# tsadja/ShaSTA

Hardware: AMD Instinct MI355X
Metric: affinity frame-pairs/sec at N=M=500, F=256 (higher is better)
Workload: dtype f32; 1 GPU; synthetic N=M=500, F=256 (num_point 4 x C 64), nf=7: affinity forward from HBM-resident NHWC BEV maps (SURVEY 8a rows 4-16); max_obj=500, num_feats=7, num_point=4, arithmetic=f16x2, parallelism=replica x1

## Files before the change

### shasta_amd/csrc/pair.hip

```cpp
#include "stages.hpp"
#include "pair_lane.hpp"

namespace shasta {

struct PackArgs {
    shasta_linear fs[4], fd[3], rc[3], aff0;
    float* out;
    int N, nf, F;
};

__device__ __forceinline__ void layer_src(const PackArgs& a, int l, const float*& W, const float*& b, int& ldw) {
    const PairDims d(a.F);
    switch (l) {
        case L_FS2: W = a.fs[1].weight; b = a.fs[1].bias; ldw = d.H1; break;
        case L_FS3: W = a.fs[2].weight; b = a.fs[2].bias; ldw = d.H2; break;
        case L_FS4: W = a.fs[3].weight; b = a.fs[3].bias; ldw = d.H3; break;
        case L_RC2: W = a.rc[1].weight; b = a.rc[1].bias; ldw = d.R1; break;
        case L_RC3: W = a.rc[2].weight; b = a.rc[2].bias; ldw = d.R2; break;
        case L_FD2: W = a.fd[1].weight; b = a.fd[1].bias; ldw = 32; break;
        default:    W = a.fd[2].weight; b = a.fd[2].bias; ldw = 8; break;
    }
}

__global__ void pack_pair_weights_kernel(PackArgs a) {
    const PackedLayout P(a.N, a.nf, a.F);
    const PairDims d(a.F);
    const int tid = blockIdx.x * blockDim.x + threadIdx.x;
    const int nth = gridDim.x * blockDim.x;
    const int F = a.F, nf = a.nf;
    for (int l = 0; l < L_COUNT; ++l) {
        const LayerDesc L = layer_desc(F, l);
        const float *W, *b;
        int ldw;
        layer_src(a, l, W, b, ldw);
        const int nob = a4_nob(F, l), kg = a4_kg(F, l);
        float* o = a.out + P.a4 + a4_offset(F, l);
        for (int e = tid; e < nob * kg * 16; e += nth) {
            const int kk = e & 3, i = (e >> 2) & 3, g = (e >> 4) % kg, ob = (e >> 4) / kg;
            const int f = 4 * ob + i, k = 4 * g + kk;
            o[e] = (f < L.hout && k < L.kin) ? W[(size_t)f * ldw + k] : 0.0f;
        }
        for (int e = tid; e < nob * 4; e += nth) o[nob * kg * 16 + e] = e < L.hout ? b[e] : 0.0f;
    }
    const int E12 = P.E12;
    for (int e = tid; e < E12 * F; e += nth) {
        const int j = e / F, k = e % F;
        float wp, wc;
        if (j < d.H1) {
            wp = a.fs[0].weight[(size_t)j * 2 * F + k];
            wc = a.fs[0].weight[(size_t)j * 2 * F + F + k];
        } else {
            const size_t row = (size_t)(j - d.H1) * (2 * F + 2 * nf);
            wp = a.rc[0].weight[row + k];
            wc = a.rc[0].weight[row + F + nf + k];
        }
        a.out[P.wemb_prev + e] = wp;
        a.out[P.wemb_cur + e] = wc;
    }
    for (int e = tid; e < (E12 + 3) / 4 * 4; e += nth)
        a.out[P.bemb_cur + e] = e < d.H1 ? a.fs[0].bias[e] : (e < E12 ? a.rc[0].bias[e - d.H1] : 0.0f);
    for (int e = tid; e < (d.R1 + 32) * 8; e += nth) {
        const int j = e >> 3, c = e & 7;
        float wp = 0.0f, wc = 0.0f;
        if (c < nf) {
            if (j < d.R1) {
                const size_t row = (size_t)j * (2 * F + 2 * nf);
                wp = a.rc[0].weight[row + F + c];
                wc = a.rc[0].weight[row + 2 * F + nf + c];
            } else {
                const size_t row = (size_t)(j - d.R1) * (2 * nf);
                wp = a.fd[0].weight[row + c];
                wc = a.fd[0].weight[row + nf + c];
            }
        }
        a.out[P.wbox_prev + e] = wp;
        a.out[P.wbox_cur + e] = wc;
    }
    for (int e = tid; e < 32; e += nth) a.out[P.bbox_cur + e] = a.fd[0].bias[e];
    for (int e = tid; e < 128 * P.Dp; e += nth) {
        const int j = e / P.Dp, k = e % P.Dp;
        a.out[P.aff0 + e] = k < P.D ? a.aff0.weight[(size_t)j * P.D + k] : 0.0f;
    }
}

struct RowPrepArgs {
    const float* packed;
    const float* tab[2];
    float* emb[2];
    float* hand[2];
    float* denom;
    int B, T, N, nf, F, nrow_blocks, nhand_blocks, dblocks, dper;
};

template <int ND, int NF>
__device__ __forceinline__ void col_norm_block(const RowPrepArgs& a, int cb, int tid) {
    const int T = a.T, D = a.T, nf = NF ? NF : a.nf;
    const int b = cb / a.dblocks, dl = tid & 15, tg = tid >> 4;
    const int d0 = (cb % a.dblocks) * (16 * ND) + dl;
    float db[ND][7];
#pragma unroll
    for (int j = 0; j < ND; ++j) {
        const f32x4* h = reinterpret_cast<const f32x4*>(a.tab[1] + ((size_t)b * D + min(d0 + 16 * j, D - 1)) * 8);
        const f32x4 x = h[0], c = h[1];
        db[j][0] = x[0]; db[j][1] = x[1]; db[j][2] = x[2]; db[j][3] = x[3]; db[j][4] = c[0]; db[j][5] = c[1]; db[j][6] = c[2];
#pragma unroll
        for (int k = 0; k < 7; ++k)
            if (k >= nf) db[j][k] = 0.0f;
    }
    __shared__ __attribute__((aligned(16))) f32x4 sp[2 * 512];
    const f32x4* hp = reinterpret_cast<const f32x4*>(a.tab[0] + (size_t)b * T * 8);
    typedef float f2 __attribute__((ext_vector_type(2)));
    f2 ssq2[ND];
#pragma unroll
    for (int j = 0; j < ND; ++j) ssq2[j] = f2{0.0f, 0.0f};
    for (int t0 = 0; t0 < T; t0 += 512) {
        const int nt = min(512, T - t0);
        if (t0) __syncthreads();
        for (int e = tid; e < 2 * nt; e += 256) {
            f32x4 v = hp[(size_t)t0 * 2 + e];
            const int k0 = (e & 1) * 4;
#pragma unroll
            for (int q = 0; q < 4; ++q)
                if (k0 + q >= nf) v[q] = 0.0f;
            sp[e] = v;
        }
        __syncthreads();
        for (int t = tg; t < nt; t += 32) {
            const int tb = t + 16;
            const bool two = tb < nt;
            const f32x4 x0 = sp[2 * t], c0 = sp[2 * t + 1];
            const f32x4 x1 = sp[2 * (two ? tb : t)], c1 = sp[2 * (two ? tb : t) + 1];
            const f2 p[7] = {f2{x0[0], x1[0]}, f2{x0[1], x1[1]}, f2{x0[2], x1[2]}, f2{x0[3], x1[3]}, f2{c0[0], c1[0]}, f2{c0[1], c1[1]},
                             f2{c0[2], c1[2]}};
#pragma unroll
            for (int j = 0; j < ND; ++j) {
                f2 d2 = {0.0f, 0.0f};
#pragma unroll
                for (int k = 0; k < (NF ? NF : 7); ++k) {
                    const f2 df = p[k] - f2{db[j][k], db[j][k]};
                    d2 += df * df;
                }
                f2 sq = d2 * d2;
                if (!two) sq[1] = 0.0f;
                ssq2[j] += sq;
            }
        }
    }
    __shared__ float red4[ND][16][17];
#pragma unroll
    for (int j = 0; j < ND; ++j) red4[j][dl][tg] = ssq2[j][0] + ssq2[j][1];
    __syncthreads();
    if (tid < 16 * ND) {
        const int j = tid >> 4, l = tid & 15, dd = (cb % a.dblocks) * (16 * ND) + 16 * j + l;
        if (dd < D) {
            float tot = 0.0f;
#pragma unroll
            for (int i = 0; i < 16; ++i) tot += red4[j][l][i];
            a.denom[(size_t)b * D + dd] = fmaxf(sqrtf(tot), 1e-12f);
        }
    }
}

__global__ __launch_bounds__(256) void col_norm_kernel(RowPrepArgs a) { col_norm_block<4, 0>(a, blockIdx.x, threadIdx.x); }

__global__ __launch_bounds__(256) void row_prep_kernel(RowPrepArgs a) {
    const int tid = threadIdx.x;
    if ((int)blockIdx.x < a.nrow_blocks) {
        __shared__ __attribute__((aligned(16))) float wT[7 * 104];
        const PackedLayout P(a.N, a.nf, a.F);
        const PairDims d(a.F);
        const int J = d.R1 + 32;
        const int half = a.nrow_blocks / 2;
        const int which = (int)blockIdx.x >= half;
        const int side_row0 = (blockIdx.x - which * half) * 32;
        {
            const float* wb = a.packed + (which ? P.wbox_cur : P.wbox_prev);
            for (int e = tid; e < J * 8; e += 256) {
                const int j = e >> 3, c = e & 7;
                if (c < 7) wT[c * 104 + j] = wb[e];
            }
        }
        __syncthreads();
        const int q = tid & 31, nq = J / 4;
        for (int it = 0; it < 4; ++it) {
            const int row = side_row0 + it * 8 + (tid >> 5);
            if (row >= a.B * a.T) continue;
            float amax = 0.0f;
            if (q < nq) {
                const f32x4* bp = reinterpret_cast<const f32x4*>(a.tab[which] + (size_t)row * 8);
                const f32x4 b0 = bp[0], b1 = bp[1];
                const float bx[7] = {b0[0], b0[1], b0[2], b0[3], b1[0], b1[1], b1[2]};
                f32x4 s = {0.0f, 0.0f, 0.0f, 0.0f};
#pragma unroll
                for (int c = 0; c < 7; ++c) {
                    const f32x4 w4 = *reinterpret_cast<const f32x4*>(&wT[c * 104 + 4 * q]);
                    s[0] = fmaf(w4[0], bx[c], s[0]); s[1] = fmaf(w4[1], bx[c], s[1]);
                    s[2] = fmaf(w4[2], bx[c], s[2]); s[3] = fmaf(w4[3], bx[c], s[3]);
                }
                f32x4* e = reinterpret_cast<f32x4*>(a.emb[which] + (size_t)row * d.ET + d.H1 + 4 * q);
                const int j = 4 * q;
                if (j < d.R1) {
                    f32x4 v = *e;
                    s[0] += v[0]; s[1] += v[1]; s[2] += v[2]; s[3] += v[3];
                } else if (which) {
                    const f32x4 bb = *reinterpret_cast<const f32x4*>(a.packed + P.bbox_cur + (j - d.R1));
                    s[0] += bb[0]; s[1] += bb[1]; s[2] += bb[2]; s[3] += bb[3];
                }
                *e = s;
                amax = absmax_keep_nan(absmax_keep_nan(fabsf(s[0]), fabsf(s[1])), absmax_keep_nan(fabsf(s[2]), fabsf(s[3])));
            } else {
                const f32x4* e = reinterpret_cast<const f32x4*>(a.emb[which] + (size_t)row * d.ET);
                for (int c4 = q - nq; c4 < d.H1 / 4; c4 += 32 - nq) {
                    const f32x4 v = e[c4];
                    amax = absmax_keep_nan(amax, absmax_keep_nan(absmax_keep_nan(fabsf(v[0]), fabsf(v[1])), absmax_keep_nan(fabsf(v[2]), fabsf(v[3]))));
                }
            }
#pragma unroll
            for (int off = 16; off > 0; off >>= 1) amax = absmax_keep_nan(amax, __shfl_xor(amax, off, 64));
            if (q == 0) a.hand[which][(size_t)row * 16 + 13] = amax;
        }
        return;
    }
    if ((int)blockIdx.x < a.nrow_blocks + a.nhand_blocks) {
        const int item = (blockIdx.x - a.nrow_blocks) * 256 + tid;
        if (item >= 2 * a.B * a.T) return;
        const int which = item / (a.B * a.T), row = item % (a.B * a.T);
        const f32x4* bp = reinterpret_cast<const f32x4*>(a.tab[which] + (size_t)row * 8);
        const f32x4 b0 = bp[0], b1 = bp[1];
        f32x4* h = reinterpret_cast<f32x4*>(a.hand[which] + (size_t)row * 16);
        const int nf = a.nf;
        h[0] = f32x4{b0[0], nf > 1 ? b0[1] : 0.0f, nf > 2 ? b0[2] : 0.0f, nf > 3 ? b0[3] : 0.0f};
        h[1] = f32x4{nf > 4 ? b1[0] : 0.0f, nf > 5 ? b1[1] : 0.0f, nf > 6 ? b1[2] : 0.0f, 0.0f};
        h[2] = f32x4{logf(b0[3] + 1e-10f), logf(b1[0] + 1e-10f), logf(b1[1] + 1e-10f), cosf(b1[2])};
        a.hand[which][(size_t)row * 16 + 12] = sinf(b1[2]);
        return;
    }
    const int cb = blockIdx.x - a.nrow_blocks - a.nhand_blocks;
    if (a.dper == 4) {
        col_norm_block<4, 0>(a, cb, tid);
    } else {
        col_norm_block<1, 0>(a, cb, tid);
    }
}

template <int F, int WPB, int DT>
struct PairMfma4Lds {
    static constexpr int US = PairDims(F).ET + 4;
    static constexpr int RING = 3 * (64 / DT);
    static constexpr int uc = 0;
    static constexpr int a4 = uc + DT * US;
    static constexpr int up = a4 + pad4(a4_total(F));
    static constexpr size_t bytes = (size_t)(up + WPB * RING * UP_SLOT) * sizeof(float);
};
static_assert(PairMfma4Lds<64, 8, 64>::bytes == 49760 && PairMfma4Lds<64, 8, 32>::bytes == 63584 &&
              PairMfma4Lds<256, 8, 64>::bytes == 66800 && PairMfma4Lds<256, 8, 32>::bytes == 74480 &&
              PairMfma4Lds<320, 8, 64>::bytes == 74336 && PairMfma4Lds<320, 8, 32>::bytes == 79968, "the sizes the launcher spelt out before");

template <int F, int WPB, int DT = 64>
__global__ __launch_bounds__(64 * WPB) __attribute__((amdgpu_waves_per_eu(4))) void pair_mfma4_kernel(const float* __restrict__ packed, const float* __restrict__ UP,
                                                         const float* __restrict__ UC, const float* __restrict__ hand_prev,
                                                         const float* __restrict__ hand_det, const float* __restrict__ denom,
                                                         float* __restrict__ residual, int T, int D, int ld, int nf,
                                                         int TW) {
    constexpr PairDims dm(F);
    constexpr int H1 = dm.H1, R1 = dm.R1, ET = dm.ET;
    using Lds = PairMfma4Lds<F, WPB, DT>;
    constexpr int US = Lds::US, RING = Lds::RING;
    static_assert(DT == 64 || DT == 32, "64 detections x 1 track or 32 detections x 2 tracks per wave");
    constexpr int TPI = 64 / DT;
    extern __shared__ __attribute__((aligned(16))) float s_dyn4[];
    float* s_uc = s_dyn4 + Lds::uc;
    float* s_a4 = s_dyn4 + Lds::a4;
    float* s_up = s_dyn4 + Lds::up;
    const int tid = threadIdx.x, lane = tid & 63;
    const int wid = __builtin_amdgcn_readfirstlane(tid >> 6);
    const int dlane = lane & (DT - 1), th = lane / DT;
    int lbx, lby, b;
    xcd_logical_block(lbx, lby, b);
    const int d0 = lbx * DT;
    const int d = d0 + dlane, dcl = min(d, D - 1);
    {
        const f32x4* src = reinterpret_cast<const f32x4*>(UC);
#pragma unroll 4
        for (int e = tid; e < DT * (ET / 4); e += 64 * WPB) {
            const int r = e / (ET / 4), c = e - r * (ET / 4);
            *reinterpret_cast<f32x4*>(&s_uc[r * US + 4 * c]) = src[((size_t)b * D + min(d0 + r, D - 1)) * (ET / 4) + c];
        }
        a4_stage<F, 64 * WPB>(packed, s_a4, tid);
    }
    float hd[12];
    (void)load_hand_det(hand_det + ((size_t)b * D + dcl) * 16, hd);
    const float dnm = denom[(size_t)b * D + dcl], rdn = 1.0f / dnm;
    __syncthreads();
    const float* ucrow = s_uc + dlane * US;
    const A4Lane a4l(s_a4, lane);

    const int t_beg = (lby * WPB + wid) * TW;
    const int t_end = min(T, t_beg + TW);
    float* my_up = s_up + wid * (RING * UP_SLOT);
    const bool hp_lane = lane >= ET / 4 && lane < ET / 4 + 4;
    const int up_lane = 4 * min(lane, ET / 4 - 1), hp_off = 4 * (lane - ET / 4);
    auto dma_up = [&](int row, int slot) {
        const size_t r = (size_t)b * T + min(row, T - 1);
        const float* src = hp_lane ? hand_prev + r * 16 + hp_off : UP + r * ET + up_lane;
        __builtin_amdgcn_global_load_lds((const __attribute__((address_space(1))) void*)src,
                                         (__attribute__((address_space(3))) void*)(my_up + slot * UP_SLOT), 16, 0, 0);
    };
    if (t_beg < t_end) {
#pragma unroll
        for (int i = 0; i < 2 * TPI; ++i) dma_up(t_beg + i, i);
    }
    for (int t = t_beg; t < t_end; t += TPI) {
        asm volatile("s_waitcnt vmcnt(0)" ::: "memory");
#pragma unroll
        for (int i = 0; i < TPI; ++i) dma_up(t + 2 * TPI + i, (t - t_beg + 2 * TPI + i) % RING);
        const int tt = t + th;
        unsigned upo = (unsigned)(unsigned long long)(my_up + ((t - t_beg + th) % RING) * UP_SLOT);
        asm volatile("" : "+v"(upo));
        const lfloat* up = (const lfloat*)(unsigned long long)upo;
        float hp[16];
        {
            const f32x4 h0 = *reinterpret_cast<const lf32x4*>(up + ET), h1 = *reinterpret_cast<const lf32x4*>(up + ET + 4),
                        h2 = *reinterpret_cast<const lf32x4*>(up + ET + 8), h3 = *reinterpret_cast<const lf32x4*>(up + ET + 12);
#pragma unroll
            for (int k = 0; k < 4; ++k) {
                hp[k] = h0[k];
                hp[4 + k] = h1[k];
                hp[8 + k] = h2[k];
                hp[12 + k] = h3[k];
            }
        }
        const lfloat *arow, *abias;
        a4l.per_track(arow, abias);

        auto layer12 = [&](auto tag, int seg, f32x4* acc) {
            using AL = decltype(tag);
            a4_init<AL>(abias, acc);
#pragma unroll
            for (int kg = 0; kg < AL::KG; ++kg) {
                const f32x4 u = *reinterpret_cast<const f32x4*>(ucrow + seg + 4 * kg);
                const f32x4 upv = *reinterpret_cast<const lf32x4*>(up + seg + 4 * kg);
                f32x4 a4[AL::NOB];
#pragma unroll
                for (int ob = 0; ob < AL::NOB; ++ob) a4[ob] = *reinterpret_cast<const lf32x4*>(arow + AL::OFF + (ob * AL::KG + kg) * 16);
#pragma unroll
                for (int kk = 0; kk < 4; ++kk) {
                    if (4 * kg + kk < AL::KIN) {
                        const float h = relu_nan(upv[kk] + u[kk]);
#pragma unroll
                        for (int ob = 0; ob < AL::NOB; ++ob) acc[ob] = MFMA4(a4[ob][kk], h, acc[ob]);
                    }
                }
            }
        };
        f32x4 a_rc2[A4<F, L_RC2>::NOB], a_rc3[A4<F, L_RC3>::NOB];
        f32x4 a_fs2[A4<F, L_FS2>::NOB], a_fs3[A4<F, L_FS3>::NOB], a_fs4[A4<F, L_FS4>::NOB];
        f32x4 a_fd2[A4<F, L_FD2>::NOB], a_fd3[A4<F, L_FD3>::NOB];
        layer12(A4<F, L_RC2>{}, H1, a_rc2);
        layer12(A4<F, L_FS2>{}, 0, a_fs2);
        layer12(A4<F, L_FD2>{}, H1 + R1, a_fd2);
        a4_layer<A4<F, L_RC3>, A4_RELU_NAN>(arow, abias, a_rc2, a_rc3);
        a4_layer<A4<F, L_FS3>, A4_RELU_NAN>(arow, abias, a_fs2, a_fs3);
        a4_layer<A4<F, L_FD3>, A4_RELU_NAN>(arow, abias, a_fd2, a_fd3);
        a4_layer<A4<F, L_FS4>, A4_RELU_NAN>(arow, abias, a_fs3, a_fs4);

        const float dist = hand_dist(hp, hd, dnm, rdn);
        const float res = pair_combine(a_rc3[0], a_fd3[0][0], dist, a_fs4[0][0]);
        if (d < D && tt < t_end) residual[((size_t)b * T + tt) * ld + d] = res;
    }
}

int pair_residual(const shasta_weights* w, const float* packed, int B, const float* feat, const float* prev_feat,
                  const float* det_tab, const float* prev_tab, float* residual, int ld, void* ws, size_t ws_bytes,
                  hipStream_t st, hipEvent_t ev0, hipEvent_t ev1) {
    const int N = w->max_obj, F = w->feat_dim, nf = w->num_feats, T = N + 2, D = N + 2;
    const PairDims d(F);
    const PackedLayout P(N, nf, F);
    const PairWs L(B, N, F);
    if (ws_bytes < L.total) {
        set_error_msg("pair_residual: workspace too small");
        return SHASTA_E_WORKSPACE;
    }
    if (B == 0) return SHASTA_OK;
    char* base = static_cast<char*>(ws);
    float* UP = reinterpret_cast<float*>(base + L.up);
    float* UC = reinterpret_cast<float*>(base + L.uc);
    float* hand_prev = reinterpret_cast<float*>(base + L.hand_prev);
    float* hand_det = reinterpret_cast<float*>(base + L.hand_det);
    float* denom = reinterpret_cast<float*>(base + L.denom);

    const bool gemm_f32 = (w->options & SHASTA_OPT_F32_EMBED_GEMM) != 0;
    const bool fused = B * T >= 8192 && !gemm_f32 && embed_rows_serves(F) && ((uintptr_t)feat | (uintptr_t)prev_feat) % 16 == 0;
    int rc;
    if (fused)
        rc = launch_embed_rows(w, packed, prev_feat, feat, prev_tab, det_tab, UP, UC, hand_prev, hand_det, B * T, st);
    else
        rc = launch_gemm_nt_dual(prev_feat, packed + P.wemb_prev, nullptr, UP, feat, packed + P.wemb_cur, packed + P.bemb_cur, UC, F, F,
                                 d.ET, B * T, P.E12, F, 0, st);
    if (rc) return rc;
    RowPrepArgs rp;
    rp.packed = packed;
    rp.tab[0] = prev_tab;
    rp.tab[1] = det_tab;
    rp.emb[0] = UP;
    rp.emb[1] = UC;
    rp.hand[0] = hand_prev;
    rp.hand[1] = hand_det;
    rp.denom = denom;
    rp.B = B;
    rp.T = T;
    rp.N = N;
    rp.nf = nf;
    rp.F = F;
    rp.nrow_blocks = fused ? 0 : 2 * cdiv(B * T, 32);
    rp.nhand_blocks = cdiv(2 * B * T, 256);
    rp.dper = cdiv(D, 16) * B >= 2048 ? 4 : 1;
    rp.dblocks = cdiv(D, 16 * rp.dper);
    if (rp.dper == 4) {
        hipLaunchKernelGGL(row_prep_kernel, dim3(rp.nrow_blocks + rp.nhand_blocks), dim3(256), 0, st, rp);
        rc = check_launch("row_prep");
        if (rc) return rc;
        hipLaunchKernelGGL(col_norm_kernel, dim3(rp.dblocks * B), dim3(256), 0, st, rp);
        rc = check_launch("col_norm");
    } else {
        hipLaunchKernelGGL(row_prep_kernel, dim3(rp.nrow_blocks + rp.nhand_blocks + rp.dblocks * B), dim3(256), 0, st, rp);
        rc = check_launch("row_prep");
    }
    if (rc) return rc;
    if ((w->options & SHASTA_OPT_F16X2_PAIR) && F == 256) {
        if (ev0) (void)hipEventRecord(ev0, st);
        const bool grid = (w->options & SHASTA_OPT_F16GRID_PAIR) != 0 && fused;
        rc = launch_pair_f16(packed, packed + P.p16, UP, UC, hand_prev, hand_det, denom, residual, B, T, D, ld, nf, grid, st);
        if (ev1) (void)hipEventRecord(ev1, st);
        return rc;
    }
    if ((w->options & SHASTA_OPT_F16X2_PAIR) && pair_f16w_serves(F)) {
        if (ev0) (void)hipEventRecord(ev0, st);
        rc = launch_pair_f16w(packed, packed + P.p16w, UP, UC, hand_prev, hand_det, denom, residual, B, T, D, ld, F, st);
        if (ev1) (void)hipEventRecord(ev1, st);
        if (rc != SHASTA_E_UNSUPPORTED) return rc;
    }
    constexpr int wpb = 8;
    const double fill64 = (double)D / (64.0 * cdiv(D, 64)), fill32 = (double)D / (32.0 * cdiv(D, 32));
    const int dt = fill32 > 1.1 * fill64 ? 32 : 64, tpi = 64 / dt;
    int ny = 1;
    while ((long)B * cdiv(D, dt) * ny < 1024 && cdiv(T, wpb * ny * 2) >= 2 * tpi) ny *= 2;
    while ((long)B * cdiv(D, dt) * ny < 256 && cdiv(T, wpb * ny * 2) >= tpi) ny *= 2;
    const int tw = cdiv(cdiv(T, wpb * ny), tpi) * tpi;
    dim3 grid(cdiv(D, dt), cdiv(T, wpb * tw), B);
#define SHASTA_LAUNCH_PAIR4_DT(FF, DD)                                                                                                    \
    do {                                                                                                                                  \
        constexpr size_t lds = PairMfma4Lds<FF, wpb, DD>::bytes;                                                                          \
        if (lds > 64 * 1024)                                                                                                              \
            (void)hipFuncSetAttribute((const void*)pair_mfma4_kernel<FF, wpb, DD>, hipFuncAttributeMaxDynamicSharedMemorySize, (int)lds); \
        hipLaunchKernelGGL((pair_mfma4_kernel<FF, wpb, DD>), grid, dim3(64 * wpb), lds, st, packed, UP, UC, hand_prev, hand_det, denom,   \
                           residual, T, D, ld, nf, tw);                                                                                   \
    } while (0)
#define SHASTA_LAUNCH_PAIR4(FF)                 \
    do {                                        \
        if (dt == 32) SHASTA_LAUNCH_PAIR4_DT(FF, 32); \
        else SHASTA_LAUNCH_PAIR4_DT(FF, 64);    \
    } while (0)
    if (ev0) (void)hipEventRecord(ev0, st);
    switch (F) {
        case 64: SHASTA_LAUNCH_PAIR4(64); break;
        case 256: SHASTA_LAUNCH_PAIR4(256); break;
        case 320: SHASTA_LAUNCH_PAIR4(320); break;
        default: set_error_msg("pair_residual: feat_dim must be 64, 256 or 320"); return SHASTA_E_ARG;
    }
    if (ev1) (void)hipEventRecord(ev1, st);
#undef SHASTA_LAUNCH_PAIR4_DT
#undef SHASTA_LAUNCH_PAIR4
    return check_launch("pair_mfma4");
}

int pack_weights(const shasta_weights* w, float* packed, hipStream_t st) {
    PackArgs a;
    for (int i = 0; i < 4; ++i) a.fs[i] = w->fuse_shape[i];
    for (int i = 0; i < 3; ++i) a.fd[i] = w->fuse_det[i];
    for (int i = 0; i < 3; ++i) a.rc[i] = w->res_coeff[i];
    a.aff0 = w->aff[0];
    a.out = packed;
    a.N = w->max_obj;
    a.nf = w->num_feats;
    a.F = w->feat_dim;
    hipLaunchKernelGGL(pack_pair_weights_kernel, dim3(256), dim3(256), 0, st, a);
    int rc = check_launch("pack_pair_weights");
    if (rc) return rc;
    const PackedLayout P(w->max_obj, w->num_feats, w->feat_dim);
    if ((rc = aff_pieces_pack(w, packed + P.affp, st))) return rc;
    if ((rc = aff_f16_pack(w, packed + P.aff16, st))) return rc;
    if (w->feat_dim == 256 && (rc = pair_f16_pack(w, packed + P.p16, st))) return rc;
    if (pair_f16w_serves(w->feat_dim) && (rc = pair_f16w_pack(w, packed + P.p16w, st))) return rc;
    if (embed_rows_serves(w->feat_dim) && (rc = embed_pack(w, packed, st))) return rc;
    return rc;
}

}
```

### shasta_amd/csrc/pair_f16.hip

```cpp
#include "stages.hpp"
#include "pair_lane.hpp"
#include "pieces.hpp"

namespace shasta {


constexpr int P16_FRAG_DW = 2 * 4 * 64 * 4;

__global__ __launch_bounds__(256) void pair_f16_pack_kernel(PairF16PackArgs a) {
    __shared__ float red[3][4];
    __shared__ int ex[3];
    const int tid = threadIdx.x;
    const float* W[3] = {a.w_fs2, a.w_rc2, a.w_fd2};
    const int cnt[3] = {16 * 32, 16 * 64, 8 * 32};
    pair2_range_exponents(W, cnt, a.out, P16_FRAG_DW, red, ex);
    const int lane = tid & 63, frag = tid >> 6;
    const int i = lane & 15, kb = lane >> 4;
    const int mlp = frag == 0 ? 0 : frag == 3 ? 2 : 1;
    const int rows = mlp == 2 ? 8 : 16, kin = mlp == 1 ? 64 : 32, ks = frag == 2 ? 1 : 0;
    float v[8];
#pragma unroll
    for (int j = 0; j < 8; ++j) v[j] = i < rows ? __builtin_ldexpf(W[mlp][i * kin + 32 * ks + 8 * kb + j], ex[mlp]) : 0.0f;
    store_weight_pieces(v, a.out, 4, frag, lane);
}

int pair_f16_pack(const shasta_weights* w, float* out, hipStream_t st) {
    hipLaunchKernelGGL(pair_f16_pack_kernel, dim3(1), dim3(256), 0, st, pair_f16_pack_args(w, out));
    return check_launch("pair_f16_pack");
}

constexpr int PF_TS = 44;
constexpr int GR_ROW = 136;

template <int WPB, bool GRID>
struct PairF16Lds {
    static constexpr int US = PairDims(256).ET + 4;
    static constexpr int uc = 0;
    static constexpr int ucl = uc + 64 * (GR_ROW / 2);
    static constexpr int a4 = uc + (GRID ? 2 * 64 * (GR_ROW / 2) : 64 * US);
    static constexpr int up = a4 + pad4(a4_total(256));
    static constexpr int tr = up + WPB * 3 * UP_SLOT;
    static constexpr int upp = tr + WPB * 64 * PF_TS;
    static constexpr size_t bytes = (size_t)(upp + (GRID ? WPB * 128 : 0)) * sizeof(float);
};
static_assert(PairF16Lds<8, false>::bytes == 156912 && PairF16Lds<8, true>::bytes == 162032, "the sizes the launcher spelt out before");


template <int WPB, bool GRID>
__global__ __launch_bounds__(64 * WPB) void pair_f16_kernel(const float* __restrict__ packed, const uint32_t* __restrict__ p16,
                                                       const float* __restrict__ UP, const float* __restrict__ UC,
                                                       const float* __restrict__ hand_prev, const float* __restrict__ hand_det,
                                                       const float* __restrict__ denom, float* __restrict__ residual, int T,
                                                       int D, int ld, int nf, int TWG, int TA, int TB) {
    constexpr int F = 256;
    constexpr PairDims dm(F);
    constexpr int ET = dm.ET;
    static_assert(dm.H1 == 32 && dm.R1 == 64 && ET == 128 && dm.H2 == 16 && dm.R2 == 16, "pair_f16_kernel is laid out for F = 256");
    using Lds = PairF16Lds<WPB, GRID>;
    constexpr int US = Lds::US;
    extern __shared__ __attribute__((aligned(16))) float s_dynh[];
    float* s_uc = s_dynh + Lds::uc;
    float* s_a4 = s_dynh + Lds::a4;
    float* s_up = s_dynh + Lds::up;
    float* s_tr = s_dynh + Lds::tr;
    uint32_t* s_uch = reinterpret_cast<uint32_t*>(s_dynh + Lds::uc);
    uint32_t* s_ucl = reinterpret_cast<uint32_t*>(s_dynh + Lds::ucl);
    uint32_t* s_upp = reinterpret_cast<uint32_t*>(s_dynh + Lds::upp);
    const int tid = threadIdx.x, lane = tid & 63;
    const int wid = __builtin_amdgcn_readfirstlane(tid >> 6);
    int lbx, by, b;
    xcd_logical_block(lbx, by, b);
    const int d0 = lbx * 64;
    const int d = d0 + lane, dcl = min(d, D - 1);
    {
        if constexpr (!GRID) {
            const f32x4* src = reinterpret_cast<const f32x4*>(UC);
#pragma unroll 4
            for (int e = tid; e < 64 * (ET / 4); e += 64 * WPB) {
                const int r = e / (ET / 4), c = e - r * (ET / 4);
                const int cp = (((c >> 1) & 1) << 4) | (((c >> 2) & 1) << 3) | ((c >> 3) << 1) | (c & 1);
                *reinterpret_cast<f32x4*>(&s_uc[r * US + 4 * cp]) = src[((size_t)b * D + min(d0 + r, D - 1)) * (ET / 4) + c];
            }
        }
        a4_stage<F, 64 * WPB>(packed, s_a4, tid);
    }
    float hd[12];
    float mc = load_hand_det(hand_det + ((size_t)b * D + dcl) * 16, hd);
#pragma unroll
    for (int off = 32; off > 0; off >>= 1) mc = absmax_keep_nan(mc, __shfl_xor(mc, off, 64));
    const float dnm = denom[(size_t)b * D + dcl], rdn = 1.0f / dnm;
    int ge[3] = {0, 0, 0};
    bool grid_finite = true;
    if constexpr (GRID) {
        float mcr[3], mur[3] = {0.0f, 0.0f, 0.0f};
        {
            const float* h = hand_det + ((size_t)b * D + dcl) * 16;
            mcr[0] = h[14];
            mcr[1] = h[15];
            mcr[2] = h[13];
        }
        const int tw0 = by * TWG, tw1 = min(T, tw0 + TWG);
        for (int t = tw0 + tid; t < tw1; t += 64 * WPB) {
            const float* h = hand_prev + ((size_t)b * T + t) * 16;
            mur[0] = absmax_keep_nan(mur[0], h[14]);
            mur[1] = absmax_keep_nan(mur[1], h[15]);
            mur[2] = absmax_keep_nan(mur[2], h[13]);
        }
#pragma unroll
        for (int r = 0; r < 3; ++r)
#pragma unroll
            for (int off = 32; off > 0; off >>= 1) {
                mcr[r] = absmax_keep_nan(mcr[r], __shfl_xor(mcr[r], off, 64));
                mur[r] = absmax_keep_nan(mur[r], __shfl_xor(mur[r], off, 64));
            }
        float* red = s_tr;
        if (lane == 0) {
            red[wid * 3 + 0] = mur[0];
            red[wid * 3 + 1] = mur[1];
            red[wid * 3 + 2] = mur[2];
        }
        __syncthreads();
#pragma unroll
        for (int r = 0; r < 3; ++r) {
            float m = red[r];
            for (int w = 1; w < WPB; ++w) m = absmax_keep_nan(m, red[w * 3 + r]);
            const float bound = (m + mcr[r]) * 1.002f;
            grid_finite = grid_finite && (bound < INFINITY);
            ge[r] = range_exponent_bits(__float_as_uint(bound)) - 3;
        }
        __syncthreads();
        const f32x4* src = reinterpret_cast<const f32x4*>(UC);
        for (int e = tid; e < 64 * (ET / 4); e += 64 * WPB) {
            const int r = e / (ET / 4), c = e - r * (ET / 4);
            const f32x4 v = src[((size_t)b * D + min(d0 + r, D - 1)) * (ET / 4) + c];
            const int ex = c < 8 ? ge[0] : c < 24 ? ge[1] : ge[2];
            _Float16 hh[4], ll[4];
#pragma unroll
            for (int q = 0; q < 4; ++q) {
                const float sv = __builtin_ldexpf(v[q], ex), hi = rintf(sv);
                hh[q] = (_Float16)hi;
                ll[q] = (_Float16)(rintf((sv - hi) * 2048.0f) * (1.0f / 2048.0f));
            }
            typedef uint32_t pu2 __attribute__((ext_vector_type(2)));
            typedef _Float16 ph2t __attribute__((ext_vector_type(2)));
            *reinterpret_cast<pu2*>(s_uch + r * (GR_ROW / 2) + 2 * c) =
                pu2{__builtin_bit_cast(uint32_t, ph2t{hh[0], hh[1]}), __builtin_bit_cast(uint32_t, ph2t{hh[2], hh[3]})};
            *reinterpret_cast<pu2*>(s_ucl + r * (GR_ROW / 2) + 2 * c) =
                pu2{__builtin_bit_cast(uint32_t, ph2t{ll[0], ll[1]}), __builtin_bit_cast(uint32_t, ph2t{ll[2], ll[3]})};
        }
    }
    u32x4 wh[4], wl[4];
#pragma unroll
    for (int f = 0; f < 4; ++f) {
        wh[f] = reinterpret_cast<const u32x4*>(p16)[(0 * 4 + f) * 64 + lane];
        wl[f] = reinterpret_cast<const u32x4*>(p16)[(1 * 4 + f) * 64 + lane];
    }
    const int ew_fs = reinterpret_cast<const int*>(p16)[P16_FRAG_DW + 0], ew_rc = reinterpret_cast<const int*>(p16)[P16_FRAG_DW + 1],
              ew_fd = reinterpret_cast<const int*>(p16)[P16_FRAG_DW + 2];
    __syncthreads();
    const A4Lane a4l(s_a4, lane);
    const f32x4 zero4 = {0, 0, 0, 0};
    const int p = lane & 15, kb = lane >> 4;
    float* my_tr = s_tr + wid * (64 * PF_TS);

    const int t_beg = by * TWG + (wid < 4 ? wid * TA : 4 * TA + (wid - 4) * TB);
    const int t_end = min(min(T, (by + 1) * TWG), t_beg + (wid < 4 ? TA : TB));
    float* my_up = s_up + wid * (3 * UP_SLOT);
    const bool hp_lane = lane >= ET / 4 && lane < ET / 4 + 4;
    const int up_lane = 4 * min(lane, ET / 4 - 1), hp_off = 4 * (lane - ET / 4);
    auto dma_up = [&](int row, int slot) {
        const size_t r = (size_t)b * T + min(row, T - 1);
        const float* src = hp_lane ? hand_prev + r * 16 + hp_off : UP + r * ET + up_lane;
        __builtin_amdgcn_global_load_lds((const __attribute__((address_space(1))) void*)src,
                                         (__attribute__((address_space(3))) void*)(my_up + slot * UP_SLOT), 16, 0, 0);
    };
    if (t_beg < t_end) {
        dma_up(t_beg, 0);
        dma_up(t_beg + 1, 1);
    }
    for (int t = t_beg; t < t_end; ++t) {
        asm volatile("s_waitcnt vmcnt(0)" ::: "memory");
        dma_up(t + 2, (t - t_beg + 2) % 3);
        unsigned upo = (unsigned)(unsigned long long)(my_up + ((t - t_beg) % 3) * UP_SLOT);
        asm volatile("" : "+v"(upo));
        const lfloat* up = (const lfloat*)(unsigned long long)upo;
        float hp[16];
        {
            const f32x4 h0 = *reinterpret_cast<const lf32x4*>(up + ET), h1 = *reinterpret_cast<const lf32x4*>(up + ET + 4),
                        h2 = *reinterpret_cast<const lf32x4*>(up + ET + 8), h3 = *reinterpret_cast<const lf32x4*>(up + ET + 12);
#pragma unroll
            for (int k = 0; k < 4; ++k) {
                hp[k] = h0[k];
                hp[4 + k] = h1[k];
                hp[8 + k] = h2[k];
                hp[12 + k] = h3[k];
            }
        }
        typedef _Float16 ph2 __attribute__((ext_vector_type(2)));
        bool finite_bound;
        int e1 = 0;
        f32x2 cs2 = {0.0f, 0.0f};
        const f32x2 c14 = {16384.0f, 16384.0f};
        f32x2 upv[GRID ? 1 : 16];
        u32x4 uph[GRID ? 4 : 1], upl[GRID ? 4 : 1];
        if constexpr (!GRID) {
            const float bound = hp[13] + mc;
            finite_bound = bound < INFINITY;
            e1 = range_exponent_bits(__float_as_uint(bound));
            const float cs = __builtin_ldexpf(1.0f, e1 - 14);
            cs2 = f32x2{cs, cs};
#pragma unroll
            for (int s = 0; s < 4; ++s) {
                const f32x4 a = *reinterpret_cast<const lf32x4*>(up + 32 * s + 8 * kb), c = *reinterpret_cast<const lf32x4*>(up + 32 * s + 8 * kb + 4);
                upv[4 * s] = f32x2{a[0], a[1]} * cs2;
                upv[4 * s + 1] = f32x2{a[2], a[3]} * cs2;
                upv[4 * s + 2] = f32x2{c[0], c[1]} * cs2;
                upv[4 * s + 3] = f32x2{c[2], c[3]} * cs2;
            }
        } else {
            finite_bound = grid_finite;
            uint32_t* my_p = s_upp + wid * 128;
            {
                typedef __attribute__((address_space(3))) f32x2 lf32x2;
                const f32x2 v = *reinterpret_cast<const lf32x2*>(up + 2 * lane);
                const int ex = lane < 16 ? ge[0] : lane < 48 ? ge[1] : ge[2];
                const float s0 = __builtin_ldexpf(v[0], ex), s1 = __builtin_ldexpf(v[1], ex);
                const float h0 = rintf(s0), h1v = rintf(s1);
                const ph2 hh = {(_Float16)h0, (_Float16)h1v};
                const ph2 ll = {(_Float16)(rintf((s0 - h0) * 2048.0f) * (1.0f / 2048.0f)), (_Float16)(rintf((s1 - h1v) * 2048.0f) * (1.0f / 2048.0f))};
                my_p[lane] = __builtin_bit_cast(uint32_t, hh);
                my_p[64 + lane] = __builtin_bit_cast(uint32_t, ll);
            }
#pragma unroll
            for (int s = 0; s < 4; ++s) {
                uph[s] = *reinterpret_cast<const u32x4*>(my_p + 16 * s + 4 * kb);
                upl[s] = *reinterpret_cast<const u32x4*>(my_p + 64 + 16 * s + 4 * kb);
            }
        }
        auto load_uc = [&](int sub, f32x4 (&u)[8]) {
            if constexpr (GRID) {
                const uint32_t* hr = s_uch + (16 * sub + p) * (GR_ROW / 2) + 4 * kb;
                const uint32_t* lr = s_ucl + (16 * sub + p) * (GR_ROW / 2) + 4 * kb;
#pragma unroll
                for (int s = 0; s < 4; ++s) {
                    u[s] = __builtin_bit_cast(f32x4, *reinterpret_cast<const u32x4*>(hr + 16 * s));
                    u[4 + s] = __builtin_bit_cast(f32x4, *reinterpret_cast<const u32x4*>(lr + 16 * s));
                }
                return;
            }
            const float* ucr = s_uc + (16 * sub + p) * US + ((kb & 1) << 6) + ((kb >> 1) << 5);
#pragma unroll
            for (int s = 0; s < 4; ++s) {
                u[2 * s] = *reinterpret_cast<const f32x4*>(ucr + 8 * s);
                u[2 * s + 1] = *reinterpret_cast<const f32x4*>(ucr + 8 * s + 4);
            }
        };
        auto cut = [&](const f32x4 (&u)[8], u32x4 (&xh)[4], u32x4 (&xl)[4]) {
            if constexpr (GRID) {
                const _Float16 m1 = (_Float16)-1.0f;
                const f16x8 neg1 = {m1, m1, m1, m1, m1, m1, m1, m1};
#pragma unroll
                for (int s = 0; s < 4; ++s) {
                    const f16x8 h = __builtin_bit_cast(f16x8, u[s]) + __builtin_bit_cast(f16x8, uph[s]);
                    const f16x8 l = __builtin_bit_cast(f16x8, u[4 + s]) + __builtin_bit_cast(f16x8, upl[s]);
                    const f16x8 h2 = __builtin_elementwise_max(h, neg1);
                    const f16x8 l2 = __builtin_elementwise_max(l, -h2);
                    xh[s] = __builtin_bit_cast(u32x4, h2);
                    xl[s] = __builtin_bit_cast(u32x4, l2);
                }
                return;
            }
#pragma unroll
            for (int s = 0; s < 4; ++s) {
#pragma unroll
                for (int j2 = 0; j2 < 2; ++j2) {
                    const f32x4 uu = u[2 * s + j2];
                    const f32x2 sa = fma2_relu01(f32x2{uu[0], uu[1]}, cs2, upv[4 * s + 2 * j2]) * c14;
                    const f32x2 sb = fma2_relu01(f32x2{uu[2], uu[3]}, cs2, upv[4 * s + 2 * j2 + 1]) * c14;
                    const uint32_t hA = cvt_f16x2(sa[0], sa[1]), hB = cvt_f16x2(sb[0], sb[1]);
                    xh[s][2 * j2] = hA;
                    xh[s][2 * j2 + 1] = hB;
                    xl[s][2 * j2] = cvt_f16x2(f16_res_lo(sa[0], hA), f16_res_hi(sa[1], hA));
                    xl[s][2 * j2 + 1] = cvt_f16x2(f16_res_lo(sb[0], hB), f16_res_hi(sb[1], hB));
                }
            }
        };
        auto mma = [&](const u32x4 (&xh)[4], const u32x4 (&xl)[4], f32x4& a_fs, f32x4& a_rc, f32x4& a_fd) {
            a_fs = a_rc = a_fd = zero4;
            a_fs = mfma_16x16x32_f16(wl[0], xh[0], a_fs);
            a_rc = mfma_16x16x32_f16(wl[1], xh[1], a_rc);
            a_fd = mfma_16x16x32_f16(wl[3], xh[3], a_fd);
            a_fs = mfma_16x16x32_f16(wh[0], xl[0], a_fs);
            a_rc = mfma_16x16x32_f16(wh[1], xl[1], a_rc);
            a_fd = mfma_16x16x32_f16(wh[3], xl[3], a_fd);
            a_rc = mfma_16x16x32_f16(wl[2], xh[2], a_rc);
            a_fs = mfma_16x16x32_f16(wh[0], xh[0], a_fs);
            a_fd = mfma_16x16x32_f16(wh[3], xh[3], a_fd);
            a_rc = mfma_16x16x32_f16(wh[2], xl[2], a_rc);
            a_rc = mfma_16x16x32_f16(wh[1], xh[1], a_rc);
            a_rc = mfma_16x16x32_f16(wh[2], xh[2], a_rc);
        };
        auto store = [&](int sub, const f32x4& a_fs, const f32x4& a_rc, const f32x4& a_fd) {
            float* row = my_tr + (16 * sub + p) * PF_TS + 4 * kb;
            *reinterpret_cast<f32x4*>(row) = a_rc;
            *reinterpret_cast<f32x4*>(row + 16) = a_fs;
            if (kb < 2) *reinterpret_cast<f32x4*>(row + 32) = a_fd;
        };
        {
            f32x4 ua[8], ub[8];
            u32x4 xha[4], xla[4], xhb[4], xlb[4];
            f32x4 fsA, rcA, fdA, fsB, rcB, fdB;
            load_uc(0, ua);
            load_uc(1, ub);
            cut(ua, xha, xla);
            load_uc(2, ua);
            cut(ub, xhb, xlb);
            mma(xha, xla, fsA, rcA, fdA);
            store(0, fsA, rcA, fdA);
            load_uc(3, ub);
            cut(ua, xha, xla);
            mma(xhb, xlb, fsB, rcB, fdB);
            store(1, fsB, rcB, fdB);
            cut(ub, xhb, xlb);
            mma(xha, xla, fsA, rcA, fdA);
            store(2, fsA, rcA, fdA);
            mma(xhb, xlb, fsB, rcB, fdB);
            store(3, fsB, rcB, fdB);
        }
        const lfloat *arow, *abias;
        a4l.per_track(arow, abias);
        const float i_rc = __builtin_ldexpf(1.0f, -((GRID ? ge[1] : e1) + ew_rc)), i_fs = __builtin_ldexpf(1.0f, -((GRID ? ge[0] : e1) + ew_fs)),
                    i_fd = __builtin_ldexpf(1.0f, -((GRID ? ge[2] : e1) + ew_fd));
        f32x4 a_rc2[4], a_fs2[4], a_fd2[2];
        {
            const float* mine = my_tr + lane * PF_TS;
            const float* b_rc = s_a4 + A4<F, L_RC2>::OFF + A4<F, L_RC2>::BIAS;
            const float* b_fs = s_a4 + A4<F, L_FS2>::OFF + A4<F, L_FS2>::BIAS;
            const float* b_fd = s_a4 + A4<F, L_FD2>::OFF + A4<F, L_FD2>::BIAS;
#pragma unroll
            for (int g = 0; g < 4; ++g) {
                a_rc2[g] = a4_descale_relu(*reinterpret_cast<const f32x4*>(mine + 4 * g), i_rc, *reinterpret_cast<const f32x4*>(b_rc + 4 * g));
                a_fs2[g] = a4_descale_relu(*reinterpret_cast<const f32x4*>(mine + 16 + 4 * g), i_fs, *reinterpret_cast<const f32x4*>(b_fs + 4 * g));
            }
#pragma unroll
            for (int g = 0; g < 2; ++g)
                a_fd2[g] = a4_descale_relu(*reinterpret_cast<const f32x4*>(mine + 32 + 4 * g), i_fd, *reinterpret_cast<const f32x4*>(b_fd + 4 * g));
        }
        asm volatile("" : "+v"(a_rc2[0]), "+v"(a_rc2[1]), "+v"(a_rc2[2]), "+v"(a_rc2[3]), "+v"(a_fs2[0]), "+v"(a_fs2[1]), "+v"(a_fs2[2]),
                     "+v"(a_fs2[3]), "+v"(a_fd2[0]), "+v"(a_fd2[1]));
        f32x4 a_rc3[A4<F, L_RC3>::NOB], a_fs3[A4<F, L_FS3>::NOB], a_fs4[A4<F, L_FS4>::NOB], a_fd3[A4<F, L_FD3>::NOB];
        {
            using RC = A4<F, L_RC3>;
            using FS = A4<F, L_FS3>;
            using FD = A4<F, L_FD3>;
            static_assert(RC::NOB == 1 && FS::NOB == 2 && FD::NOB == 1 && RC::KG == 4 && FS::KG == 4 && FD::KG == 2, "F = 256");
            a4_init<RC>(abias, a_rc3);
            a4_init<FS>(abias, a_fs3);
            a4_init<FD>(abias, a_fd3);
#pragma unroll
            for (int kg = 0; kg < 4; ++kg) {
                const f32x4 w_rc = *reinterpret_cast<const lf32x4*>(arow + RC::OFF + kg * 16);
                const f32x4 w_f0 = *reinterpret_cast<const lf32x4*>(arow + FS::OFF + kg * 16);
                const f32x4 w_f1 = *reinterpret_cast<const lf32x4*>(arow + FS::OFF + (FS::KG + kg) * 16);
                f32x4 w_fd = zero4;
                if (kg < 2) w_fd = *reinterpret_cast<const lf32x4*>(arow + FD::OFF + kg * 16);
#pragma unroll
                for (int kk = 0; kk < 4; ++kk) {
                    a_rc3[0] = MFMA4(w_rc[kk], a_rc2[kg][kk], a_rc3[0]);
                    a_fs3[0] = MFMA4(w_f0[kk], a_fs2[kg][kk], a_fs3[0]);
                    a_fs3[1] = MFMA4(w_f1[kk], a_fs2[kg][kk], a_fs3[1]);
                    if (kg < 2) a_fd3[0] = MFMA4(w_fd[kk], a_fd2[kg][kk], a_fd3[0]);
                }
            }
        }
        a4_layer<A4<F, L_FS4>, A4_RELU_FMAX>(arow, abias, a_fs3, a_fs4);

        const float dist = hand_dist(hp, hd, dnm, rdn);
        const float res = pair_combine(a_rc3[0], a_fd3[0][0], dist, a_fs4[0][0]);
        if (d < D) residual[((size_t)b * T + t) * ld + d] = finite_bound ? res : __builtin_nanf("");
    }
}

int launch_pair_f16(const float* packed, const float* p16, const float* UP, const float* UC, const float* hand_prev,
                    const float* hand_det, const float* denom, float* residual, int B, int T, int D, int ld, int nf, bool grid,
                    hipStream_t st) {
    constexpr int wpb = 8;
    int ny = 1;
    while ((long)B * cdiv(D, 64) * ny < 512 && cdiv(T, wpb * ny * 2) >= 2) ny *= 2;
    const int twg = cdiv(cdiv(T, ny), wpb) * wpb;
    int ta = twg / wpb, tb = ta;
    if (wpb == 8) {
        const int per_simd = twg / 4;
        ta = (per_simd * 1000 + (1000 + 615) / 2) / (1000 + 615);
        tb = per_simd - ta;
    }
    const size_t lds = grid ? PairF16Lds<wpb, true>::bytes : PairF16Lds<wpb, false>::bytes;
    dim3 grd(cdiv(D, 64), cdiv(T, twg), B);
    if (grid) {
        (void)hipFuncSetAttribute((const void*)pair_f16_kernel<wpb, true>, hipFuncAttributeMaxDynamicSharedMemorySize, (int)lds);
        hipLaunchKernelGGL((pair_f16_kernel<wpb, true>), grd, dim3(64 * wpb), lds, st, packed, reinterpret_cast<const uint32_t*>(p16), UP, UC,
                           hand_prev, hand_det, denom, residual, T, D, ld, nf, twg, ta, tb);
    } else {
        (void)hipFuncSetAttribute((const void*)pair_f16_kernel<wpb, false>, hipFuncAttributeMaxDynamicSharedMemorySize, (int)lds);
        hipLaunchKernelGGL((pair_f16_kernel<wpb, false>), grd, dim3(64 * wpb), lds, st, packed, reinterpret_cast<const uint32_t*>(p16), UP, UC,
                           hand_prev, hand_det, denom, residual, T, D, ld, nf, twg, ta, tb);
    }
    return check_launch("pair_f16");
}

}
```

### shasta_amd/csrc/stages.hpp

```cpp
#pragma once
#include "common.hpp"
#include "pair_layout.hpp"

namespace shasta {

size_t bev_absmax_slot_bytes(int items);
int launch_absmax_finalize(const unsigned* slots, unsigned* out, int items, hipStream_t st);
int launch_bev_gather(const float* bev, int B, int H, int W, int C, const float* boxes, int N, int box_stride, int box_batch_stride,
                      int num_point, float pc_x0, float pc_y0, float vs_x, float vs_y, float out_stride, float* out, int out_row_stride,
                      int out_batch_stride, unsigned* absmax, hipStream_t st, const float* bev2 = nullptr, const float* boxes2 = nullptr,
                      float* out2 = nullptr, unsigned* absmax2 = nullptr);

int launch_gemm_nt_dual(const float* A0, const float* W0, const float* bias0, float* C0, const float* A1, const float* W1,
                        const float* bias1, float* C1, int lda, int ldw, int ldc, int M, int N, int K, int act, hipStream_t st);
int launch_gemm_nt_quad(const float* const A[4], const float* const W[4], const float* const bias[4], float* const C[4], int lda,
                        int ldw, int ldc, int M, int N, int K, int act, hipStream_t st);
bool gemm_nt_quad_direct_ok(const float* const A[4], const float* const W[4], int lda, int ldw, int K);

int launch_anchor_l1_mfma(const float* const W[4], const float* feat, const float* prev_feat, float* part, int H, int K, int B,
                          int x_batch_stride, int* ks_out, hipStream_t st);

int launch_x_maxima(const float* feat, const float* prev_feat, int K, int B, int x_batch_stride, unsigned* xmax, hipStream_t st);
int launch_w_maxima(const float* const W[4], int H, int K, unsigned* wmax, float* sumabs, hipStream_t st);
size_t precut_image_bytes(int H, int K);
int launch_precut_weights(const float* const W[4], const unsigned* wmax, void* img, int H, int K, hipStream_t st);
size_t anchor_split_workspace_bytes(int B, int K);
bool anchor_split_serves(int B, int K, int x_batch_stride);
void launch_split_x(const float* feat, const float* prev_feat, void* xs, int K, int B, int x_batch_stride, int np, const unsigned* xmax,
                    bool precut, hipStream_t st);
void launch_anchor_l1_split(const float* const W[4], const void* xs, float* part, int H, int K, int B, int* ks_out, int np,
                            const unsigned* wmax, const void* wimg, hipStream_t st);

int anchor_shape(const shasta_weights* w, int B, float* feat, float* prev_feat, void* ws, size_t ws_bytes, hipStream_t st,
                 hipEvent_t ev0, hipEvent_t ev1, const unsigned* wmax, bool xmax_ready);
bool anchor_shape_uses_xmax(const shasta_weights* w, int B);
int anchor_boxes(const shasta_weights* w, int B, float* det_boxes, const float* prev_det_boxes, int box_stride, float* det_tab,
                 float* prev_tab, float* hid_ws, hipStream_t st, float* anchors_out);
bool anchor_stage_fused_serves(const shasta_weights* w, int B);
int anchor_stage_fused(const shasta_weights* w, int B, float* feat, float* prev_feat, float* det_boxes, const float* prev_det_boxes,
                       int box_stride, float* det_tab, float* prev_tab, void* ws, size_t ws_bytes, hipStream_t st, hipEvent_t ev0,
                       hipEvent_t ev1, const unsigned* wmax, bool xmax_ready, float* anchors_out);

int pair_f16_pack(const shasta_weights* w, float* out, hipStream_t st);
int launch_pair_f16(const float* packed, const float* p16, const float* UP, const float* UC, const float* hand_prev,
                    const float* hand_det, const float* denom, float* residual, int B, int T, int D, int ld, int nf, bool grid,
                    hipStream_t st);
bool pair_f16w_serves(int F);
int pair_f16w_pack(const shasta_weights* w, float* out, hipStream_t st);
int launch_pair_f16w(const float* packed, const float* p16, const float* UP, const float* UC, const float* hand_prev,
                     const float* hand_det, const float* denom, float* residual, int B, int T, int D, int ld, int F, hipStream_t st);

int embed_pack(const shasta_weights* w, float* packed, hipStream_t st);
bool embed_rows_serves(int F);
int launch_embed_rows(const shasta_weights* w, const float* packed, const float* prev_feat, const float* feat, const float* prev_tab,
                      const float* det_tab, float* UP, float* UC, float* hand_prev, float* hand_det, int M, hipStream_t st);

int pair_residual(const shasta_weights* w, const float* packed, int B, const float* feat, const float* prev_feat, const float* det_tab,
                  const float* prev_tab, float* residual, int ld, void* ws, size_t ws_bytes, hipStream_t st, hipEvent_t ev0,
                  hipEvent_t ev1);
int pack_weights(const shasta_weights* w, float* packed, hipStream_t st);

int aff_pieces_pack(const shasta_weights* w, float* out, hipStream_t st);
int aff_f16_pack(const shasta_weights* w, float* out, hipStream_t st);
bool aff_pieces_serves(int D);
int launch_aff_pieces(const shasta_weights* w, const float* packed_pieces, const float* residual, int ld, float* matched, int ldm,
                      float* m1, int M, hipStream_t st);
int launch_aff_frame(const shasta_weights* w, const float* packed_pieces, const float* residual, int ld, float* matched, int ldm, float* m1,
                     float* m2, int B, void* ws, hipStream_t st);
int launch_aff_frame16(const shasta_weights* w, const float* packed16, const float* residual, int ld, float* matched, int ldm, float* m1,
                       float* m2, int B, void* ws, hipStream_t st);

int aff_status(const shasta_weights* w, int B, int ld, const void* ws, int* status, hipStream_t st);
int aff_softmax(const shasta_weights* w, const float* packed, int B, const float* residual, int ld, float* m1, float* m2,
                float* matched_out, void* ws, size_t ws_bytes, hipStream_t st);


inline size_t ws_take(size_t& o, size_t bytes) {
    const size_t at = o;
    o += align_up(bytes, 256);
    return at;
}

struct AnchorShapeWs {
    size_t part, hidden, xs, xmax, wmax, slots, total;
    AnchorShapeWs(int B, int N, int F) {
        const size_t H = (size_t)N * F / 64;
        size_t o = 0;
        part = ws_take(o, (size_t)64 * B * 4 * H * sizeof(float));
        hidden = ws_take(o, (size_t)B * 4 * H * sizeof(float));
        xs = ws_take(o, anchor_split_workspace_bytes(B, N * F));
        xmax = ws_take(o, (size_t)2 * B * sizeof(unsigned));
        wmax = ws_take(o, (size_t)4 * H * sizeof(unsigned));
        slots = o;
        total = o + bev_absmax_slot_bytes(2 * B);
    }
};

struct AnchorBoxesWs {
    size_t hid, x7, total;
    AnchorBoxesWs(int B, int N) {
        const int HD = 7 * N / 32;
        size_t o = 0;
        hid = ws_take(o, (size_t)B * 4 * (HD > 1 ? HD : 1) * sizeof(float));
        x7 = ws_take(o, (size_t)2 * B * pad4(7 * N) * sizeof(float));
        total = o;
    }
};

struct PairWs {
    size_t up, uc, hand_prev, hand_det, denom, total;
    PairWs(int B, int N, int F) {
        const size_t rows = (size_t)B * (N + 2);
        size_t o = 0;
        up = ws_take(o, rows * PairDims(F).ET * sizeof(float));
        uc = ws_take(o, rows * PairDims(F).ET * sizeof(float));
        hand_prev = ws_take(o, rows * 16 * sizeof(float));
        hand_det = ws_take(o, rows * 16 * sizeof(float));
        denom = ws_take(o, rows * sizeof(float));
        total = o;
    }
};

struct AffWs {
    size_t matched, ctrl, part, total;
    AffWs(int B, int N) {
        const int T = N + 2;
        size_t o = 0;
        matched = ws_take(o, (size_t)B * T * pad4(T) * sizeof(float));
        ctrl = ws_take(o, (size_t)(B + 2) * sizeof(unsigned));
        part = ws_take(o, (size_t)B * cdiv(T, 64) * 1024 * sizeof(float));
        total = o;
    }
};

}
```

Measured before the change: 64280 frame-pairs/s.

## Make f16 pair kernel persistent with per-XCD atomic tile tickets

Turns the f16x2 pair kernel into a persistent kernel with one workgroup per CU when there are more tiles than CUs. Workgroups take tiles from eight atomic ticket counters, one per XCD-sized slice, and steal from other slices once their own runs out. Packed weights are staged into LDS once per workgroup instead of once per tile. The cost is a global atomic and an extra barrier per tile, plus counters that row_prep must reset on every call.

```diff
diff --git a/shasta_amd/csrc/pair.hip b/shasta_amd/csrc/pair.hip
--- a/shasta_amd/csrc/pair.hip
+++ b/shasta_amd/csrc/pair.hip
@@ -89,6 +89,7 @@
     float* emb[2];
     float* hand[2];
     float* denom;
+    unsigned* tickets;
     int B, T, N, nf, F, nrow_blocks, nhand_blocks, dblocks, dper;
 };
 
@@ -223,6 +224,7 @@
     }
     if ((int)blockIdx.x < a.nrow_blocks + a.nhand_blocks) {
         const int item = (blockIdx.x - a.nrow_blocks) * 256 + tid;
+        if (item < 8) a.tickets[item] = 0;
         if (item >= 2 * a.B * a.T) return;
         const int which = item / (a.B * a.T), row = item % (a.B * a.T);
         const f32x4* bp = reinterpret_cast<const f32x4*>(a.tab[which] + (size_t)row * 8);
@@ -407,6 +409,7 @@
     rp.hand[0] = hand_prev;
     rp.hand[1] = hand_det;
     rp.denom = denom;
+    rp.tickets = reinterpret_cast<unsigned*>(base + L.tickets);
     rp.B = B;
     rp.T = T;
     rp.N = N;
@@ -430,7 +433,7 @@
     if ((w->options & SHASTA_OPT_F16X2_PAIR) && F == 256) {
         if (ev0) (void)hipEventRecord(ev0, st);
         const bool grid = (w->options & SHASTA_OPT_F16GRID_PAIR) != 0 && fused;
-        rc = launch_pair_f16(packed, packed + P.p16, UP, UC, hand_prev, hand_det, denom, residual, B, T, D, ld, nf, grid, st);
+        rc = launch_pair_f16(packed, packed + P.p16, UP, UC, hand_prev, hand_det, denom, residual, B, T, D, ld, nf, grid, rp.tickets, st);
         if (ev1) (void)hipEventRecord(ev1, st);
         return rc;
     }
diff --git a/shasta_amd/csrc/pair_f16.hip b/shasta_amd/csrc/pair_f16.hip
--- a/shasta_amd/csrc/pair_f16.hip
+++ b/shasta_amd/csrc/pair_f16.hip
@@ -41,9 +41,10 @@
     static constexpr int up = a4 + pad4(a4_total(256));
     static constexpr int tr = up + WPB * 3 * UP_SLOT;
     static constexpr int upp = tr + WPB * 64 * PF_TS;
-    static constexpr size_t bytes = (size_t)(upp + (GRID ? WPB * 128 : 0)) * sizeof(float);
+    static constexpr int ctl = upp + (GRID ? WPB * 128 : 0);
+    static constexpr size_t bytes = (size_t)(ctl + 4) * sizeof(float);
 };
-static_assert(PairF16Lds<8, false>::bytes == 156912 && PairF16Lds<8, true>::bytes == 162032, "the sizes the launcher spelt out before");
+static_assert(PairF16Lds<8, false>::bytes == 156928 && PairF16Lds<8, true>::bytes == 162048, "one workgroup per CU (160 KB)");
 
 
 template <int WPB, bool GRID>
@@ -51,7 +52,8 @@
                                                        const float* __restrict__ UP, const float* __restrict__ UC,
                                                        const float* __restrict__ hand_prev, const float* __restrict__ hand_det,
                                                        const float* __restrict__ denom, float* __restrict__ residual, int T,
-                                                       int D, int ld, int nf, int TWG, int TA, int TB) {
+                                                       int D, int ld, int nf, int TWG, int TA, int TB, unsigned* __restrict__ tickets,
+                                                       int NX, int NY, int NT) {
     constexpr int F = 256;
     constexpr PairDims dm(F);
     constexpr int ET = dm.ET;
@@ -66,89 +68,14 @@
     uint32_t* s_uch = reinterpret_cast<uint32_t*>(s_dynh + Lds::uc);
     uint32_t* s_ucl = reinterpret_cast<uint32_t*>(s_dynh + Lds::ucl);
     uint32_t* s_upp = reinterpret_cast<uint32_t*>(s_dynh + Lds::upp);
+    unsigned* s_ctl = reinterpret_cast<unsigned*>(s_dynh + Lds::ctl);
     const int tid = threadIdx.x, lane = tid & 63;
     const int wid = __builtin_amdgcn_readfirstlane(tid >> 6);
-    int lbx, by, b;
-    xcd_logical_block(lbx, by, b);
-    const int d0 = lbx * 64;
-    const int d = d0 + lane, dcl = min(d, D - 1);
-    {
-        if constexpr (!GRID) {
-            const f32x4* src = reinterpret_cast<const f32x4*>(UC);
-#pragma unroll 4
-            for (int e = tid; e < 64 * (ET / 4); e += 64 * WPB) {
-                const int r = e / (ET / 4), c = e - r * (ET / 4);
-                const int cp = (((c >> 1) & 1) << 4) | (((c >> 2) & 1) << 3) | ((c >> 3) << 1) | (c & 1);
-                *reinterpret_cast<f32x4*>(&s_uc[r * US + 4 * cp]) = src[((size_t)b * D + min(d0 + r, D - 1)) * (ET / 4) + c];
-            }
-        }
-        a4_stage<F, 64 * WPB>(packed, s_a4, tid);
-    }
-    float hd[12];
-    float mc = load_hand_det(hand_det + ((size_t)b * D + dcl) * 16, hd);
-#pragma unroll
-    for (int off = 32; off > 0; off >>= 1) mc = absmax_keep_nan(mc, __shfl_xor(mc, off, 64));
-    const float dnm = denom[(size_t)b * D + dcl], rdn = 1.0f / dnm;
-    int ge[3] = {0, 0, 0};
-    bool grid_finite = true;
-    if constexpr (GRID) {
-        float mcr[3], mur[3] = {0.0f, 0.0f, 0.0f};
-        {
-            const float* h = hand_det + ((size_t)b * D + dcl) * 16;
-            mcr[0] = h[14];
-            mcr[1] = h[15];
-            mcr[2] = h[13];
-        }
-        const int tw0 = by * TWG, tw1 = min(T, tw0 + TWG);
-        for (int t = tw0 + tid; t < tw1; t += 64 * WPB) {
-            const float* h = hand_prev + ((size_t)b * T + t) * 16;
-            mur[0] = absmax_keep_nan(mur[0], h[14]);
-            mur[1] = absmax_keep_nan(mur[1], h[15]);
-            mur[2] = absmax_keep_nan(mur[2], h[13]);
-        }
-#pragma unroll
-        for (int r = 0; r < 3; ++r)
-#pragma unroll
-            for (int off = 32; off > 0; off >>= 1) {
-                mcr[r] = absmax_keep_nan(mcr[r], __shfl_xor(mcr[r], off, 64));
-                mur[r] = absmax_keep_nan(mur[r], __shfl_xor(mur[r], off, 64));
-            }
-        float* red = s_tr;
-        if (lane == 0) {
-            red[wid * 3 + 0] = mur[0];
-            red[wid * 3 + 1] = mur[1];
-            red[wid * 3 + 2] = mur[2];
-        }
-        __syncthreads();
-#pragma unroll
-        for (int r = 0; r < 3; ++r) {
-            float m = red[r];
-            for (int w = 1; w < WPB; ++w) m = absmax_keep_nan(m, red[w * 3 + r]);
-            const float bound = (m + mcr[r]) * 1.002f;
-            grid_finite = grid_finite && (bound < INFINITY);
-            ge[r] = range_exponent_bits(__float_as_uint(bound)) - 3;
-        }
-        __syncthreads();
-        const f32x4* src = reinterpret_cast<const f32x4*>(UC);
-        for (int e = tid; e < 64 * (ET / 4); e += 64 * WPB) {
-            const int r = e / (ET / 4), c = e - r * (ET / 4);
-            const f32x4 v = src[((size_t)b * D + min(d0 + r, D - 1)) * (ET / 4) + c];
-            const int ex = c < 8 ? ge[0] : c < 24 ? ge[1] : ge[2];
-            _Float16 hh[4], ll[4];
-#pragma unroll
-            for (int q = 0; q < 4; ++q) {
-                const float sv = __builtin_ldexpf(v[q], ex), hi = rintf(sv);
-                hh[q] = (_Float16)hi;
-                ll[q] = (_Float16)(rintf((sv - hi) * 2048.0f) * (1.0f / 2048.0f));
-            }
-            typedef uint32_t pu2 __attribute__((ext_vector_type(2)));
-            typedef _Float16 ph2t __attribute__((ext_vector_type(2)));
-            *reinterpret_cast<pu2*>(s_uch + r * (GR_ROW / 2) + 2 * c) =
-                pu2{__builtin_bit_cast(uint32_t, ph2t{hh[0], hh[1]}), __builtin_bit_cast(uint32_t, ph2t{hh[2], hh[3]})};
-            *reinterpret_cast<pu2*>(s_ucl + r * (GR_ROW / 2) + 2 * c) =
-                pu2{__builtin_bit_cast(uint32_t, ph2t{ll[0], ll[1]}), __builtin_bit_cast(uint32_t, ph2t{ll[2], ll[3]})};
-        }
-    }
+    const bool persistent = tickets != nullptr;
+    const unsigned per = (unsigned)NT >> 3;
+    unsigned tq = blockIdx.x & 7, tk = 0;
+    if (persistent && tid == 0) tk = __hip_atomic_fetch_add(tickets + tq, 1u, __ATOMIC_RELAXED, __HIP_MEMORY_SCOPE_AGENT);
+    a4_stage<F, 64 * WPB>(packed, s_a4, tid);
     u32x4 wh[4], wl[4];
 #pragma unroll
     for (int f = 0; f < 4; ++f) {
@@ -157,233 +84,334 @@
     }
     const int ew_fs = reinterpret_cast<const int*>(p16)[P16_FRAG_DW + 0], ew_rc = reinterpret_cast<const int*>(p16)[P16_FRAG_DW + 1],
               ew_fd = reinterpret_cast<const int*>(p16)[P16_FRAG_DW + 2];
-    __syncthreads();
     const A4Lane a4l(s_a4, lane);
     const f32x4 zero4 = {0, 0, 0, 0};
     const int p = lane & 15, kb = lane >> 4;
     float* my_tr = s_tr + wid * (64 * PF_TS);
-
-    const int t_beg = by * TWG + (wid < 4 ? wid * TA : 4 * TA + (wid - 4) * TB);
-    const int t_end = min(min(T, (by + 1) * TWG), t_beg + (wid < 4 ? TA : TB));
     float* my_up = s_up + wid * (3 * UP_SLOT);
     const bool hp_lane = lane >= ET / 4 && lane < ET / 4 + 4;
     const int up_lane = 4 * min(lane, ET / 4 - 1), hp_off = 4 * (lane - ET / 4);
-    auto dma_up = [&](int row, int slot) {
-        const size_t r = (size_t)b * T + min(row, T - 1);
-        const float* src = hp_lane ? hand_prev + r * 16 + hp_off : UP + r * ET + up_lane;
-        __builtin_amdgcn_global_load_lds((const __attribute__((address_space(1))) void*)src,
-                                         (__attribute__((address_space(3))) void*)(my_up + slot * UP_SLOT), 16, 0, 0);
-    };
-    if (t_beg < t_end) {
-        dma_up(t_beg, 0);
-        dma_up(t_beg + 1, 1);
-    }
-    for (int t = t_beg; t < t_end; ++t) {
-        asm volatile("s_waitcnt vmcnt(0)" ::: "memory");
-        dma_up(t + 2, (t - t_beg + 2) % 3);
-        unsigned upo = (unsigned)(unsigned long long)(my_up + ((t - t_beg) % 3) * UP_SLOT);
-        asm volatile("" : "+v"(upo));
-        const lfloat* up = (const lfloat*)(unsigned long long)upo;
-        float hp[16];
+    for (;;) {
+        int lbx, by, b;
+        if (persistent) {
+            if (tid == 0) {
+                for (int tries = 0; tk >= (tq == 7 ? (unsigned)NT - 7 * per : per) && tries < 7; ++tries) {
+                    tq = (tq + 1) & 7;
+                    tk = __hip_atomic_fetch_add(tickets + tq, 1u, __ATOMIC_RELAXED, __HIP_MEMORY_SCOPE_AGENT);
+                }
+                s_ctl[0] = tk < (tq == 7 ? (unsigned)NT - 7 * per : per) ? tq * per + tk : (unsigned)NT;
+            }
+            asm volatile("s_waitcnt vmcnt(0)" ::: "memory");
+            __syncthreads();
+            const int L = __builtin_amdgcn_readfirstlane(s_ctl[0]);
+            if (L >= NT) break;
+            lbx = L % NX;
+            by = (L / NX) % NY;
+            b = L / (NX * NY);
+        } else {
+            xcd_logical_block(lbx, by, b);
+        }
+        const int d0 = lbx * 64;
+        const int d = d0 + lane, dcl = min(d, D - 1);
         {
-            const f32x4 h0 = *reinterpret_cast<const lf32x4*>(up + ET), h1 = *reinterpret_cast<const lf32x4*>(up + ET + 4),
-                        h2 = *reinterpret_cast<const lf32x4*>(up + ET + 8), h3 = *reinterpret_cast<const lf32x4*>(up + ET + 12);
-#pragma unroll
-            for (int k = 0; k < 4; ++k) {
-                hp[k] = h0[k];
-                hp[4 + k] = h1[k];
-                hp[8 + k] = h2[k];
-                hp[12 + k] = h3[k];
-            }
-        }
-        typedef _Float16 ph2 __attribute__((ext_vector_type(2)));
-        bool finite_bound;
-        int e1 = 0;
-        f32x2 cs2 = {0.0f, 0.0f};
-        const f32x2 c14 = {16384.0f, 16384.0f};
-        f32x2 upv[GRID ? 1 : 16];
-        u32x4 uph[GRID ? 4 : 1], upl[GRID ? 4 : 1];
-        if constexpr (!GRID) {
-            const float bound = hp[13] + mc;
-            finite_bound = bound < INFINITY;
-            e1 = range_exponent_bits(__float_as_uint(bound));
-            const float cs = __builtin_ldexpf(1.0f, e1 - 14);
-            cs2 = f32x2{cs, cs};
-#pragma unroll
-            for (int s = 0; s < 4; ++s) {
-                const f32x4 a = *reinterpret_cast<const lf32x4*>(up + 32 * s + 8 * kb), c = *reinterpret_cast<const lf32x4*>(up + 32 * s + 8 * kb + 4);
-                upv[4 * s] = f32x2{a[0], a[1]} * cs2;
-                upv[4 * s + 1] = f32x2{a[2], a[3]} * cs2;
-                upv[4 * s + 2] = f32x2{c[0], c[1]} * cs2;
-                upv[4 * s + 3] = f32x2{c[2], c[3]} * cs2;
-            }
-        } else {
-            finite_bound = grid_finite;
-            uint32_t* my_p = s_upp + wid * 128;
+            if constexpr (!GRID) {
+                const f32x4* src = reinterpret_cast<const f32x4*>(UC);
+#pragma unroll 4
+                for (int e = tid; e < 64 * (ET / 4); e += 64 * WPB) {
+                    const int r = e / (ET / 4), c = e - r * (ET / 4);
+                    const int cp = (((c >> 1) & 1) << 4) | (((c >> 2) & 1) << 3) | ((c >> 3) << 1) | (c & 1);
+                    *reinterpret_cast<f32x4*>(&s_uc[r * US + 4 * cp]) = src[((size_t)b * D + min(d0 + r, D - 1)) * (ET / 4) + c];
+                }
+            }
+        }
+        float hd[12];
+        float mc = load_hand_det(hand_det + ((size_t)b * D + dcl) * 16, hd);
+#pragma unroll
+        for (int off = 32; off > 0; off >>= 1) mc = absmax_keep_nan(mc, __shfl_xor(mc, off, 64));
+        const float dnm = denom[(size_t)b * D + dcl], rdn = 1.0f / dnm;
+        int ge[3] = {0, 0, 0};
+        bool grid_finite = true;
+        if constexpr (GRID) {
+            float mcr[3], mur[3] = {0.0f, 0.0f, 0.0f};
             {
-                typedef __attribute__((address_space(3))) f32x2 lf32x2;
-                const f32x2 v = *reinterpret_cast<const lf32x2*>(up + 2 * lane);
-                const int ex = lane < 16 ? ge[0] : lane < 48 ? ge[1] : ge[2];
-                const float s0 = __builtin_ldexpf(v[0], ex), s1 = __builtin_ldexpf(v[1], ex);
-                const float h0 = rintf(s0), h1v = rintf(s1);
-                const ph2 hh = {(_Float16)h0, (_Float16)h1v};
-                const ph2 ll = {(_Float16)(rintf((s0 - h0) * 2048.0f) * (1.0f / 2048.0f)), (_Float16)(rintf((s1 - h1v) * 2048.0f) * (1.0f / 2048.0f))};
-                my_p[lane] = __builtin_bit_cast(uint32_t, hh);
-                my_p[64 + lane] = __builtin_bit_cast(uint32_t, ll);
-            }
-#pragma unroll
-            for (int s = 0; s < 4; ++s) {
-                uph[s] = *reinterpret_cast<const u32x4*>(my_p + 16 * s + 4 * kb);
-                upl[s] = *reinterpret_cast<const u32x4*>(my_p + 64 + 16 * s + 4 * kb);
-            }
-        }
-        auto load_uc = [&](int sub, f32x4 (&u)[8]) {
-            if constexpr (GRID) {
-                const uint32_t* hr = s_uch + (16 * sub + p) * (GR_ROW / 2) + 4 * kb;
-                const uint32_t* lr = s_ucl + (16 * sub + p) * (GR_ROW / 2) + 4 * kb;
+                const float* h = hand_det + ((size_t)b * D + dcl) * 16;
+                mcr[0] = h[14];
+                mcr[1] = h[15];
+                mcr[2] = h[13];
+            }
+            const int tw0 = by * TWG, tw1 = min(T, tw0 + TWG);
+            for (int t = tw0 + tid; t < tw1; t += 64 * WPB) {
+                const float* h = hand_prev + ((size_t)b * T + t) * 16;
+                mur[0] = absmax_keep_nan(mur[0], h[14]);
+                mur[1] = absmax_keep_nan(mur[1], h[15]);
+                mur[2] = absmax_keep_nan(mur[2], h[13]);
+            }
+#pragma unroll
+            for (int r = 0; r < 3; ++r)
+#pragma unroll
+                for (int off = 32; off > 0; off >>= 1) {
+                    mcr[r] = absmax_keep_nan(mcr[r], __shfl_xor(mcr[r], off, 64));
+                    mur[r] = absmax_keep_nan(mur[r], __shfl_xor(mur[r], off, 64));
+                }
+            float* red = s_tr;
+            if (lane == 0) {
+                red[wid * 3 + 0] = mur[0];
+                red[wid * 3 + 1] = mur[1];
+                red[wid * 3 + 2] = mur[2];
+            }
+            __syncthreads();
+#pragma unroll
+            for (int r = 0; r < 3; ++r) {
+                float m = red[r];
+                for (int w = 1; w < WPB; ++w) m = absmax_keep_nan(m, red[w * 3 + r]);
+                const float bound = (m + mcr[r]) * 1.002f;
+                grid_finite = grid_finite && (bound < INFINITY);
+                ge[r] = range_exponent_bits(__float_as_uint(bound)) - 3;
+            }
+            __syncthreads();
+            const f32x4* src = reinterpret_cast<const f32x4*>(UC);
+            for (int e = tid; e < 64 * (ET / 4); e += 64 * WPB) {
+                const int r = e / (ET / 4), c = e - r * (ET / 4);
+                const f32x4 v = src[((size_t)b * D + min(d0 + r, D - 1)) * (ET / 4) + c];
+                const int ex = c < 8 ? ge[0] : c < 24 ? ge[1] : ge[2];
+                _Float16 hh[4], ll[4];
+#pragma unroll
+                for (int q = 0; q < 4; ++q) {
+                    const float sv = __builtin_ldexpf(v[q], ex), hi = rintf(sv);
+                    hh[q] = (_Float16)hi;
+                    ll[q] = (_Float16)(rintf((sv - hi) * 2048.0f) * (1.0f / 2048.0f));
+                }
+                typedef uint32_t pu2 __attribute__((ext_vector_type(2)));
+                typedef _Float16 ph2t __attribute__((ext_vector_type(2)));
+                *reinterpret_cast<pu2*>(s_uch + r * (GR_ROW / 2) + 2 * c) =
+                    pu2{__builtin_bit_cast(uint32_t, ph2t{hh[0], hh[1]}), __builtin_bit_cast(uint32_t, ph2t{hh[2], hh[3]})};
+                *reinterpret_cast<pu2*>(s_ucl + r * (GR_ROW / 2) + 2 * c) =
+                    pu2{__builtin_bit_cast(uint32_t, ph2t{ll[0], ll[1]}), __builtin_bit_cast(uint32_t, ph2t{ll[2], ll[3]})};
+            }
+        }
+        __syncthreads();
+        if (persistent && tid == 0) tk = __hip_atomic_fetch_add(tickets + tq, 1u, __ATOMIC_RELAXED, __HIP_MEMORY_SCOPE_AGENT);
+
+        const int t_beg = by * TWG + (wid < 4 ? wid * TA : 4 * TA + (wid - 4) * TB);
+        const int t_end = min(min(T, (by + 1) * TWG), t_beg + (wid < 4 ? TA : TB));
+        auto dma_up = [&](int row, int slot) {
+            const size_t r = (size_t)b * T + min(row, T - 1);
+            const float* src = hp_lane ? hand_prev + r * 16 + hp_off : UP + r * ET + up_lane;
+            __builtin_amdgcn_global_load_lds((const __attribute__((address_space(1))) void*)src,
+                                             (__attribute__((address_space(3))) void*)(my_up + slot * UP_SLOT), 16, 0, 0);
+        };
+        if (t_beg < t_end) {
+            dma_up(t_beg, 0);
+            dma_up(t_beg + 1, 1);
+        }
+        for (int t = t_beg; t < t_end; ++t) {
+            asm volatile("s_waitcnt vmcnt(0)" ::: "memory");
+            dma_up(t + 2, (t - t_beg + 2) % 3);
+            unsigned upo = (unsigned)(unsigned long long)(my_up + ((t - t_beg) % 3) * UP_SLOT);
+            asm volatile("" : "+v"(upo));
+            const lfloat* up = (const lfloat*)(unsigned long long)upo;
+            float hp[16];
+            {
+                const f32x4 h0 = *reinterpret_cast<const lf32x4*>(up + ET), h1 = *reinterpret_cast<const lf32x4*>(up + ET + 4),
+                            h2 = *reinterpret_cast<const lf32x4*>(up + ET + 8), h3 = *reinterpret_cast<const lf32x4*>(up + ET + 12);
+#pragma unroll
+                for (int k = 0; k < 4; ++k) {
+                    hp[k] = h0[k];
+                    hp[4 + k] = h1[k];
+                    hp[8 + k] = h2[k];
+                    hp[12 + k] = h3[k];
+                }
+            }
+            typedef _Float16 ph2 __attribute__((ext_vector_type(2)));
+            bool finite_bound;
+            int e1 = 0;
+            f32x2 cs2 = {0.0f, 0.0f};
+            const f32x2 c14 = {16384.0f, 16384.0f};
+            f32x2 upv[GRID ? 1 : 16];
+            u32x4 uph[GRID ? 4 : 1], upl[GRID ? 4 : 1];
+            if constexpr (!GRID) {
+                const float bound = hp[13] + mc;
+                finite_bound = bound < INFINITY;
+                e1 = range_exponent_bits(__float_as_uint(bound));
+                const float cs = __builtin_ldexpf(1.0f, e1 - 14);
+                cs2 = f32x2{cs, cs};
 #pragma unroll
                 for (int s = 0; s < 4; ++s) {
-                    u[s] = __builtin_bit_cast(f32x4, *reinterpret_cast<const u32x4*>(hr + 16 * s));
-                    u[4 + s] = __builtin_bit_cast(f32x4, *reinterpret_cast<const u32x4*>(lr + 16 * s));
-                }
-                return;
-            }
-            const float* ucr = s_uc + (16 * sub + p) * US + ((kb & 1) << 6) + ((kb >> 1) << 5);
-#pragma unroll
-            for (int s = 0; s < 4; ++s) {
-                u[2 * s] = *reinterpret_cast<const f32x4*>(ucr + 8 * s);
-                u[2 * s + 1] = *reinterpret_cast<const f32x4*>(ucr + 8 * s + 4);
-            }
-        };
-        auto cut = [&](const f32x4 (&u)[8], u32x4 (&xh)[4], u32x4 (&xl)[4]) {
-            if constexpr (GRID) {
-                const _Float16 m1 = (_Float16)-1.0f;
-                const f16x8 neg1 = {m1, m1, m1, m1, m1, m1, m1, m1};
+                    const f32x4 a = *reinterpret_cast<const lf32x4*>(up + 32 * s + 8 * kb), c = *reinterpret_cast<const lf32x4*>(up + 32 * s + 8 * kb + 4);
+                    upv[4 * s] = f32x2{a[0], a[1]} * cs2;
+                    upv[4 * s + 1] = f32x2{a[2], a[3]} * cs2;
+                    upv[4 * s + 2] = f32x2{c[0], c[1]} * cs2;
+                    upv[4 * s + 3] = f32x2{c[2], c[3]} * cs2;
+                }
+            } else {
+                finite_bound = grid_finite;
+                uint32_t* my_p = s_upp + wid * 128;
+                {
+                    typedef __attribute__((address_space(3))) f32x2 lf32x2;
+                    const f32x2 v = *reinterpret_cast<const lf32x2*>(up + 2 * lane);
+                    const int ex = lane < 16 ? ge[0] : lane < 48 ? ge[1] : ge[2];
+                    const float s0 = __builtin_ldexpf(v[0], ex), s1 = __builtin_ldexpf(v[1], ex);
+                    const float h0 = rintf(s0), h1v = rintf(s1);
+                    const ph2 hh = {(_Float16)h0, (_Float16)h1v};
+                    const ph2 ll = {(_Float16)(rintf((s0 - h0) * 2048.0f) * (1.0f / 2048.0f)), (_Float16)(rintf((s1 - h1v) * 2048.0f) * (1.0f / 2048.0f))};
+                    my_p[lane] = __builtin_bit_cast(uint32_t, hh);
+                    my_p[64 + lane] = __builtin_bit_cast(uint32_t, ll);
+                }
 #pragma unroll
                 for (int s = 0; s < 4; ++s) {
-                    const f16x8 h = __builtin_bit_cast(f16x8, u[s]) + __builtin_bit_cast(f16x8, uph[s]);
-                    const f16x8 l = __builtin_bit_cast(f16x8, u[4 + s]) + __builtin_bit_cast(f16x8, upl[s]);
-                    const f16x8 h2 = __builtin_elementwise_max(h, neg1);
-                    const f16x8 l2 = __builtin_elementwise_max(l, -h2);
-                    xh[s] = __builtin_bit_cast(u32x4, h2);
-                    xl[s] = __builtin_bit_cast(u32x4, l2);
-                }
-                return;
-            }
-#pragma unroll
-            for (int s = 0; s < 4; ++s) {
-#pragma unroll
-                for (int j2 = 0; j2 < 2; ++j2) {
-                    const f32x4 uu = u[2 * s + j2];
-                    const f32x2 sa = fma2_relu01(f32x2{uu[0], uu[1]}, cs2, upv[4 * s + 2 * j2]) * c14;
-                    const f32x2 sb = fma2_relu01(f32x2{uu[2], uu[3]}, cs2, upv[4 * s + 2 * j2 + 1]) * c14;
-                    const uint32_t hA = cvt_f16x2(sa[0], sa[1]), hB = cvt_f16x2(sb[0], sb[1]);
-                    xh[s][2 * j2] = hA;
-                    xh[s][2 * j2 + 1] = hB;
-                    xl[s][2 * j2] = cvt_f16x2(f16_res_lo(sa[0], hA), f16_res_hi(sa[1], hA));
-                    xl[s][2 * j2 + 1] = cvt_f16x2(f16_res_lo(sb[0], hB), f16_res_hi(sb[1], hB));
-                }
-            }
-        };
-        auto mma = [&](const u32x4 (&xh)[4], const u32x4 (&xl)[4], f32x4& a_fs, f32x4& a_rc, f32x4& a_fd) {
-            a_fs = a_rc = a_fd = zero4;
-            a_fs = mfma_16x16x32_f16(wl[0], xh[0], a_fs);
-            a_rc = mfma_16x16x32_f16(wl[1], xh[1], a_rc);
-            a_fd = mfma_16x16x32_f16(wl[3], xh[3], a_fd);
-            a_fs = mfma_16x16x32_f16(wh[0], xl[0], a_fs);
-            a_rc = mfma_16x16x32_f16(wh[1], xl[1], a_rc);
-            a_fd = mfma_16x16x32_f16(wh[3], xl[3], a_fd);
-            a_rc = mfma_16x16x32_f16(wl[2], xh[2], a_rc);
-            a_fs = mfma_16x16x32_f16(wh[0], xh[0], a_fs);
-            a_fd = mfma_16x16x32_f16(wh[3], xh[3], a_fd);
-            a_rc = mfma_16x16x32_f16(wh[2], xl[2], a_rc);
-            a_rc = mfma_16x16x32_f16(wh[1], xh[1], a_rc);
-            a_rc = mfma_16x16x32_f16(wh[2], xh[2], a_rc);
-        };
-        auto store = [&](int sub, const f32x4& a_fs, const f32x4& a_rc, const f32x4& a_fd) {
-            float* row = my_tr + (16 * sub + p) * PF_TS + 4 * kb;
-            *reinterpret_cast<f32x4*>(row) = a_rc;
-            *reinterpret_cast<f32x4*>(row + 16) = a_fs;
-            if (kb < 2) *reinterpret_cast<f32x4*>(row + 32) = a_fd;
-        };
-        {
-            f32x4 ua[8], ub[8];
-            u32x4 xha[4], xla[4], xhb[4], xlb[4];
-            f32x4 fsA, rcA, fdA, fsB, rcB, fdB;
-            load_uc(0, ua);
-            load_uc(1, ub);
-            cut(ua, xha, xla);
-            load_uc(2, ua);
-            cut(ub, xhb, xlb);
-            mma(xha, xla, fsA, rcA, fdA);
-            store(0, fsA, rcA, fdA);
-            load_uc(3, ub);
-            cut(ua, xha, xla);
-            mma(xhb, xlb, fsB, rcB, fdB);
-            store(1, fsB, rcB, fdB);
-            cut(ub, xhb, xlb);
-            mma(xha, xla, fsA, rcA, fdA);
-            store(2, fsA, rcA, fdA);
-            mma(xhb, xlb, fsB, rcB, fdB);
-            store(3, fsB, rcB, fdB);
-        }
-        const lfloat *arow, *abias;
-        a4l.per_track(arow, abias);
-        const float i_rc = __builtin_ldexpf(1.0f, -((GRID ? ge[1] : e1) + ew_rc)), i_fs = __builtin_ldexpf(1.0f, -((GRID ? ge[0] : e1) + ew_fs)),
-                    i_fd = __builtin_ldexpf(1.0f, -((GRID ? ge[2] : e1) + ew_fd));
-        f32x4 a_rc2[4], a_fs2[4], a_fd2[2];
-        {
-            const float* mine = my_tr + lane * PF_TS;
-            const float* b_rc = s_a4 + A4<F, L_RC2>::OFF + A4<F, L_RC2>::BIAS;
-            const float* b_fs = s_a4 + A4<F, L_FS2>::OFF + A4<F, L_FS2>::BIAS;
-            const float* b_fd = s_a4 + A4<F, L_FD2>::OFF + A4<F, L_FD2>::BIAS;
-#pragma unroll
-            for (int g = 0; g < 4; ++g) {
-                a_rc2[g] = a4_descale_relu(*reinterpret_cast<const f32x4*>(mine + 4 * g), i_rc, *reinterpret_cast<const f32x4*>(b_rc + 4 * g));
-                a_fs2[g] = a4_descale_relu(*reinterpret_cast<const f32x4*>(mine + 16 + 4 * g), i_fs, *reinterpret_cast<const f32x4*>(b_fs + 4 * g));
-            }
-#pragma unroll
-            for (int g = 0; g < 2; ++g)
-                a_fd2[g] = a4_descale_relu(*reinterpret_cast<const f32x4*>(mine + 32 + 4 * g), i_fd, *reinterpret_cast<const f32x4*>(b_fd + 4 * g));
-        }
-        asm volatile("" : "+v"(a_rc2[0]), "+v"(a_rc2[1]), "+v"(a_rc2[2]), "+v"(a_rc2[3]), "+v"(a_fs2[0]), "+v"(a_fs2[1]), "+v"(a_fs2[2]),
-                     "+v"(a_fs2[3]), "+v"(a_fd2[0]), "+v"(a_fd2[1]));
-        f32x4 a_rc3[A4<F, L_RC3>::NOB], a_fs3[A4<F, L_FS3>::NOB], a_fs4[A4<F, L_FS4>::NOB], a_fd3[A4<F, L_FD3>::NOB];
-        {
-            using RC = A4<F, L_RC3>;
-            using FS = A4<F, L_FS3>;
-            using FD = A4<F, L_FD3>;
-            static_assert(RC::NOB == 1 && FS::NOB == 2 && FD::NOB == 1 && RC::KG == 4 && FS::KG == 4 && FD::KG == 2, "F = 256");
-            a4_init<RC>(abias, a_rc3);
-            a4_init<FS>(abias, a_fs3);
-            a4_init<FD>(abias, a_fd3);
-#pragma unroll
-            for (int kg = 0; kg < 4; ++kg) {
-                const f32x4 w_rc = *reinterpret_cast<const lf32x4*>(arow + RC::OFF + kg * 16);
-                const f32x4 w_f0 = *reinterpret_cast<const lf32x4*>(arow + FS::OFF + kg * 16);
-                const f32x4 w_f1 = *reinterpret_cast<const lf32x4*>(arow + FS::OFF + (FS::KG + kg) * 16);
-                f32x4 w_fd = zero4;
-                if (kg < 2) w_fd = *reinterpret_cast<const lf32x4*>(arow + FD::OFF + kg * 16);
-#pragma unroll
-                for (int kk = 0; kk < 4; ++kk) {
-                    a_rc3[0] = MFMA4(w_rc[kk], a_rc2[kg][kk], a_rc3[0]);
-                    a_fs3[0] = MFMA4(w_f0[kk], a_fs2[kg][kk], a_fs3[0]);
-                    a_fs3[1] = MFMA4(w_f1[kk], a_fs2[kg][kk], a_fs3[1]);
-                    if (kg < 2) a_fd3[0] = MFMA4(w_fd[kk], a_fd2[kg][kk], a_fd3[0]);
-                }
-            }
-        }
-        a4_layer<A4<F, L_FS4>, A4_RELU_FMAX>(arow, abias, a_fs3, a_fs4);
-
-        const float dist = hand_dist(hp, hd, dnm, rdn);
-        const float res = pair_combine(a_rc3[0], a_fd3[0][0], dist, a_fs4[0][0]);
-        if (d < D) residual[((size_t)b * T + t) * ld + d] = finite_bound ? res : __builtin_nanf("");
+                    uph[s] = *reinterpret_cast<const u32x4*>(my_p + 16 * s + 4 * kb);
+                    upl[s] = *reinterpret_cast<const u32x4*>(my_p + 64 + 16 * s + 4 * kb);
+                }
+            }
+            auto load_uc = [&](int sub, f32x4 (&u)[8]) {
+                if constexpr (GRID) {
+                    const uint32_t* hr = s_uch + (16 * sub + p) * (GR_ROW / 2) + 4 * kb;
+                    const uint32_t* lr = s_ucl + (16 * sub + p) * (GR_ROW / 2) + 4 * kb;
+#pragma unroll
+                    for (int s = 0; s < 4; ++s) {
+                        u[s] = __builtin_bit_cast(f32x4, *reinterpret_cast<const u32x4*>(hr + 16 * s));
+                        u[4 + s] = __builtin_bit_cast(f32x4, *reinterpret_cast<const u32x4*>(lr + 16 * s));
+                    }
+                    return;
+                }
+                const float* ucr = s_uc + (16 * sub + p) * US + ((kb & 1) << 6) + ((kb >> 1) << 5);
+#pragma unroll
+                for (int s = 0; s < 4; ++s) {
+                    u[2 * s] = *reinterpret_cast<const f32x4*>(ucr + 8 * s);
+                    u[2 * s + 1] = *reinterpret_cast<const f32x4*>(ucr + 8 * s + 4);
+                }
+            };
+            auto cut = [&](const f32x4 (&u)[8], u32x4 (&xh)[4], u32x4 (&xl)[4]) {
+                if constexpr (GRID) {
+                    const _Float16 m1 = (_Float16)-1.0f;
+                    const f16x8 neg1 = {m1, m1, m1, m1, m1, m1, m1, m1};
+#pragma unroll
+                    for (int s = 0; s < 4; ++s) {
+                        const f16x8 h = __builtin_bit_cast(f16x8, u[s]) + __builtin_bit_cast(f16x8, uph[s]);
+                        const f16x8 l = __builtin_bit_cast(f16x8, u[4 + s]) + __builtin_bit_cast(f16x8, upl[s]);
+                        const f16x8 h2 = __builtin_elementwise_max(h, neg1);
+                        const f16x8 l2 = __builtin_elementwise_max(l, -h2);
+                        xh[s] = __builtin_bit_cast(u32x4, h2);
+                        xl[s] = __builtin_bit_cast(u32x4, l2);
+                    }
+                    return;
+                }
+#pragma unroll
+                for (int s = 0; s < 4; ++s) {
+#pragma unroll
+                    for (int j2 = 0; j2 < 2; ++j2) {
+                        const f32x4 uu = u[2 * s + j2];
+                        const f32x2 sa = fma2_relu01(f32x2{uu[0], uu[1]}, cs2, upv[4 * s + 2 * j2]) * c14;
+                        const f32x2 sb = fma2_relu01(f32x2{uu[2], uu[3]}, cs2, upv[4 * s + 2 * j2 + 1]) * c14;
+                        const uint32_t hA = cvt_f16x2(sa[0], sa[1]), hB = cvt_f16x2(sb[0], sb[1]);
+                        xh[s][2 * j2] = hA;
+                        xh[s][2 * j2 + 1] = hB;
+                        xl[s][2 * j2] = cvt_f16x2(f16_res_lo(sa[0], hA), f16_res_hi(sa[1], hA));
+                        xl[s][2 * j2 + 1] = cvt_f16x2(f16_res_lo(sb[0], hB), f16_res_hi(sb[1], hB));
+                    }
+                }
+            };
+            auto mma = [&](const u32x4 (&xh)[4], const u32x4 (&xl)[4], f32x4& a_fs, f32x4& a_rc, f32x4& a_fd) {
+                a_fs = a_rc = a_fd = zero4;
+                a_fs = mfma_16x16x32_f16(wl[0], xh[0], a_fs);
+                a_rc = mfma_16x16x32_f16(wl[1], xh[1], a_rc);
+                a_fd = mfma_16x16x32_f16(wl[3], xh[3], a_fd);
+                a_fs = mfma_16x16x32_f16(wh[0], xl[0], a_fs);
+                a_rc = mfma_16x16x32_f16(wh[1], xl[1], a_rc);
+                a_fd = mfma_16x16x32_f16(wh[3], xl[3], a_fd);
+                a_rc = mfma_16x16x32_f16(wl[2], xh[2], a_rc);
+                a_fs = mfma_16x16x32_f16(wh[0], xh[0], a_fs);
+                a_fd = mfma_16x16x32_f16(wh[3], xh[3], a_fd);
+                a_rc = mfma_16x16x32_f16(wh[2], xl[2], a_rc);
+                a_rc = mfma_16x16x32_f16(wh[1], xh[1], a_rc);
+                a_rc = mfma_16x16x32_f16(wh[2], xh[2], a_rc);
+            };
+            auto store = [&](int sub, const f32x4& a_fs, const f32x4& a_rc, const f32x4& a_fd) {
+                float* row = my_tr + (16 * sub + p) * PF_TS + 4 * kb;
+                *reinterpret_cast<f32x4*>(row) = a_rc;
+                *reinterpret_cast<f32x4*>(row + 16) = a_fs;
+                if (kb < 2) *reinterpret_cast<f32x4*>(row + 32) = a_fd;
+            };
+            {
+                f32x4 ua[8], ub[8];
+                u32x4 xha[4], xla[4], xhb[4], xlb[4];
+                f32x4 fsA, rcA, fdA, fsB, rcB, fdB;
+                load_uc(0, ua);
+                load_uc(1, ub);
+                cut(ua, xha, xla);
+                load_uc(2, ua);
+                cut(ub, xhb, xlb);
+                mma(xha, xla, fsA, rcA, fdA);
+                store(0, fsA, rcA, fdA);
+                load_uc(3, ub);
+                cut(ua, xha, xla);
+                mma(xhb, xlb, fsB, rcB, fdB);
+                store(1, fsB, rcB, fdB);
+                cut(ub, xhb, xlb);
+                mma(xha, xla, fsA, rcA, fdA);
+                store(2, fsA, rcA, fdA);
+                mma(xhb, xlb, fsB, rcB, fdB);
+                store(3, fsB, rcB, fdB);
+            }
+            const lfloat *arow, *abias;
+            a4l.per_track(arow, abias);
+            const float i_rc = __builtin_ldexpf(1.0f, -((GRID ? ge[1] : e1) + ew_rc)), i_fs = __builtin_ldexpf(1.0f, -((GRID ? ge[0] : e1) + ew_fs)),
+                        i_fd = __builtin_ldexpf(1.0f, -((GRID ? ge[2] : e1) + ew_fd));
+            f32x4 a_rc2[4], a_fs2[4], a_fd2[2];
+            {
+                const float* mine = my_tr + lane * PF_TS;
+                const float* b_rc = s_a4 + A4<F, L_RC2>::OFF + A4<F, L_RC2>::BIAS;
+                const float* b_fs = s_a4 + A4<F, L_FS2>::OFF + A4<F, L_FS2>::BIAS;
+                const float* b_fd = s_a4 + A4<F, L_FD2>::OFF + A4<F, L_FD2>::BIAS;
+#pragma unroll
+                for (int g = 0; g < 4; ++g) {
+                    a_rc2[g] = a4_descale_relu(*reinterpret_cast<const f32x4*>(mine + 4 * g), i_rc, *reinterpret_cast<const f32x4*>(b_rc + 4 * g));
+                    a_fs2[g] = a4_descale_relu(*reinterpret_cast<const f32x4*>(mine + 16 + 4 * g), i_fs, *reinterpret_cast<const f32x4*>(b_fs + 4 * g));
+                }
+#pragma unroll
+                for (int g = 0; g < 2; ++g)
+                    a_fd2[g] = a4_descale_relu(*reinterpret_cast<const f32x4*>(mine + 32 + 4 * g), i_fd, *reinterpret_cast<const f32x4*>(b_fd + 4 * g));
+            }
+            asm volatile("" : "+v"(a_rc2[0]), "+v"(a_rc2[1]), "+v"(a_rc2[2]), "+v"(a_rc2[3]), "+v"(a_fs2[0]), "+v"(a_fs2[1]), "+v"(a_fs2[2]),
+                         "+v"(a_fs2[3]), "+v"(a_fd2[0]), "+v"(a_fd2[1]));
+            f32x4 a_rc3[A4<F, L_RC3>::NOB], a_fs3[A4<F, L_FS3>::NOB], a_fs4[A4<F, L_FS4>::NOB], a_fd3[A4<F, L_FD3>::NOB];
+            {
+                using RC = A4<F, L_RC3>;
+                using FS = A4<F, L_FS3>;
+                using FD = A4<F, L_FD3>;
+                static_assert(RC::NOB == 1 && FS::NOB == 2 && FD::NOB == 1 && RC::KG == 4 && FS::KG == 4 && FD::KG == 2, "F = 256");
+                a4_init<RC>(abias, a_rc3);
+                a4_init<FS>(abias, a_fs3);
+                a4_init<FD>(abias, a_fd3);
+#pragma unroll
+                for (int kg = 0; kg < 4; ++kg) {
+                    const f32x4 w_rc = *reinterpret_cast<const lf32x4*>(arow + RC::OFF + kg * 16);
+                    const f32x4 w_f0 = *reinterpret_cast<const lf32x4*>(arow + FS::OFF + kg * 16);
+                    const f32x4 w_f1 = *reinterpret_cast<const lf32x4*>(arow + FS::OFF + (FS::KG + kg) * 16);
+                    f32x4 w_fd = zero4;
+                    if (kg < 2) w_fd = *reinterpret_cast<const lf32x4*>(arow + FD::OFF + kg * 16);
+#pragma unroll
+                    for (int kk = 0; kk < 4; ++kk) {
+                        a_rc3[0] = MFMA4(w_rc[kk], a_rc2[kg][kk], a_rc3[0]);
+                        a_fs3[0] = MFMA4(w_f0[kk], a_fs2[kg][kk], a_fs3[0]);
+                        a_fs3[1] = MFMA4(w_f1[kk], a_fs2[kg][kk], a_fs3[1]);
+                        if (kg < 2) a_fd3[0] = MFMA4(w_fd[kk], a_fd2[kg][kk], a_fd3[0]);
+                    }
+                }
+            }
+            a4_layer<A4<F, L_FS4>, A4_RELU_FMAX>(arow, abias, a_fs3, a_fs4);
+
+            const float dist = hand_dist(hp, hd, dnm, rdn);
+            const float res = pair_combine(a_rc3[0], a_fd3[0][0], dist, a_fs4[0][0]);
+            if (d < D) residual[((size_t)b * T + t) * ld + d] = finite_bound ? res : __builtin_nanf("");
+        }
+        if (!persistent) break;
     }
 }
 
 int launch_pair_f16(const float* packed, const float* p16, const float* UP, const float* UC, const float* hand_prev,
                     const float* hand_det, const float* denom, float* residual, int B, int T, int D, int ld, int nf, bool grid,
-                    hipStream_t st) {
+                    unsigned* tickets, hipStream_t st) {
     constexpr int wpb = 8;
     int ny = 1;
     while ((long)B * cdiv(D, 64) * ny < 512 && cdiv(T, wpb * ny * 2) >= 2) ny *= 2;
@@ -394,17 +422,29 @@
         ta = (per_simd * 1000 + (1000 + 615) / 2) / (1000 + 615);
         tb = per_simd - ta;
     }
+    const int nx = cdiv(D, 64), nyy = cdiv(T, twg);
+    const long nt = (long)nx * nyy * B;
+    int ncu = 256;
+    {
+        int dev = 0;
+        if (hipGetDevice(&dev) == hipSuccess) {
+            int v = 0;
+            if (hipDeviceGetAttribute(&v, hipDeviceAttributeMultiprocessorCount, dev) == hipSuccess && v > 0) ncu = v;
+        }
+    }
+    const bool persistent = tickets && nt > ncu && nt < (1L << 30);
     const size_t lds = grid ? PairF16Lds<wpb, true>::bytes : PairF16Lds<wpb, false>::bytes;
-    dim3 grd(cdiv(D, 64), cdiv(T, twg), B);
-    if (grid) {
-        (void)hipFuncSetAttribute((const void*)pair_f16_kernel<wpb, true>, hipFuncAttributeMaxDynamicSharedMemorySize, (int)lds);
+    const void* fn = grid ? (const void*)pair_f16_kernel<wpb, true> : (const void*)pair_f16_kernel<wpb, false>;
+    (void)hipFuncSetAttribute(fn, hipFuncAttributeMaxDynamicSharedMemorySize, (int)lds);
+    static_assert(PairF16Lds<wpb, false>::bytes > 80 * 1024, "resident workgroups = the CUs: the LDS holds one workgroup per CU");
+    const dim3 grd = persistent ? dim3(ncu, 1, 1) : dim3(nx, nyy, B);
+    unsigned* tk = persistent ? tickets : nullptr;
+    if (grid)
         hipLaunchKernelGGL((pair_f16_kernel<wpb, true>), grd, dim3(64 * wpb), lds, st, packed, reinterpret_cast<const uint32_t*>(p16), UP, UC,
-                           hand_prev, hand_det, denom, residual, T, D, ld, nf, twg, ta, tb);
-    } else {
-        (void)hipFuncSetAttribute((const void*)pair_f16_kernel<wpb, false>, hipFuncAttributeMaxDynamicSharedMemorySize, (int)lds);
+                           hand_prev, hand_det, denom, residual, T, D, ld, nf, twg, ta, tb, tk, nx, nyy, (int)nt);
+    else
         hipLaunchKernelGGL((pair_f16_kernel<wpb, false>), grd, dim3(64 * wpb), lds, st, packed, reinterpret_cast<const uint32_t*>(p16), UP, UC,
-                           hand_prev, hand_det, denom, residual, T, D, ld, nf, twg, ta, tb);
-    }
+                           hand_prev, hand_det, denom, residual, T, D, ld, nf, twg, ta, tb, tk, nx, nyy, (int)nt);
     return check_launch("pair_f16");
 }
 
diff --git a/shasta_amd/csrc/stages.hpp b/shasta_amd/csrc/stages.hpp
--- a/shasta_amd/csrc/stages.hpp
+++ b/shasta_amd/csrc/stages.hpp
@@ -44,7 +44,7 @@
 int pair_f16_pack(const shasta_weights* w, float* out, hipStream_t st);
 int launch_pair_f16(const float* packed, const float* p16, const float* UP, const float* UC, const float* hand_prev,
                     const float* hand_det, const float* denom, float* residual, int B, int T, int D, int ld, int nf, bool grid,
-                    hipStream_t st);
+                    unsigned* tickets, hipStream_t st);
 bool pair_f16w_serves(int F);
 int pair_f16w_pack(const shasta_weights* w, float* out, hipStream_t st);
 int launch_pair_f16w(const float* packed, const float* p16, const float* UP, const float* UC, const float* hand_prev,
@@ -108,7 +108,7 @@
 };
 
 struct PairWs {
-    size_t up, uc, hand_prev, hand_det, denom, total;
+    size_t up, uc, hand_prev, hand_det, denom, tickets, total;
     PairWs(int B, int N, int F) {
         const size_t rows = (size_t)B * (N + 2);
         size_t o = 0;
@@ -117,6 +117,7 @@
         hand_prev = ws_take(o, rows * 16 * sizeof(float));
         hand_det = ws_take(o, rows * 16 * sizeof(float));
         denom = ws_take(o, rows * sizeof(float));
+        tickets = ws_take(o, 8 * sizeof(unsigned));
         total = o;
     }
 };
```

Result: slower. 63530 frame-pairs/s (-1.2%).
